# mpasha3/trips-py

Hardware: AMD Instinct MI355X
Metric: krylov_iters_per_sec (higher is better)
Workload: dtype f32; 1 GPU; blur4096_cgls; image=4096x4096 fp32, psf=Gaussian 9x9 sigma=(3,3), reflect, solver=CGLS (trips.solvers.CGLS semantics, tol=0), noise=1% Gaussian, parallelism=single

## Files before the change

include/trk.h:

```cpp
#ifndef TRK_H
#define TRK_H

#include <stdint.h>

#ifdef __cplusplus
extern "C" {
#endif

#define TRK_OK 0
#define TRK_EINVAL (-1)
#define TRK_EHIP (-2)
#define TRK_ENOMEM (-3)
#define TRK_EUNSUPPORTED (-4)
#define TRK_ENCCL (-5)

#define TRK_SQRT_NUM 1
#define TRK_SQRT_DEN 2

typedef struct trk_op trk_op;
typedef void* trk_stream;
typedef struct trk_comm trk_comm;

int trk_version(void);
const char* trk_last_error(void);
// ... 63 lines not shown
                    double* dot_out, trk_stream stream);
int trk_tv_grad_dot_xsq(trk_op* L, const float* x, const float* w, const float* r_in, double lam, float* out, const float* dotv,
                        double* dot_out, double* xsq_out, trk_stream stream);

#define TRK_HINT_OUT_FEEDS_OPPOSITE 1
#define TRK_HINT_INPUT_FROM_OPPOSITE 2
#define TRK_HINT_SUMSQ_DEFERRED 4
int trk_op_flush(trk_op* op, trk_stream stream);
int trk_op_axpby_caps(const trk_op* op, int* native);
int trk_op_apply_axpby(trk_op* op, int transpose, const float* x, double ca, const double* a_num, const double* a_den,
                       int a_flags, double cb, const double* b_num, const double* b_den, int b_flags, const float* z,
                       float* out, double* sumsq, int hints, trk_stream stream);

int trk_scalars_put(double* dst_dev, const double* src_host, int count, trk_stream stream);
typedef struct trk_mailbox trk_mailbox;
int trk_mailbox_create(int n_doubles, int slots, trk_mailbox** out);
int trk_mailbox_destroy(trk_mailbox* mb);
int trk_mailbox_host(trk_mailbox* mb, double** host_out);
int trk_mailbox_doubles(trk_mailbox* mb);
int trk_mailbox_slots(trk_mailbox* mb);
int trk_mailbox_post(trk_mailbox* mb, int slot, const double* src_dev, int offset, int count, trk_stream stream);
int trk_mailbox_wait(trk_mailbox* mb, int slot);
int trk_mailbox_post_sum(trk_mailbox* mb, int slot, const double* src_dev, int offset, int count, const double* partials,
                         int n_partials, double* sum_dev, int sum_offset, trk_stream stream);

int trk_gk_step(trk_op* op, int k, const float* u_k, const float* v_prev, float* v_k, float* u_next, double* AB, int chained,
                int defer_alpha, int defer_beta, trk_stream stream);
int trk_arnoldi_step(trk_op* op, float* V, int64_t ld, int k, float* w, double* G, int ldg, double* W, double* S, trk_stream stream);
int trk_arnoldi_step_post(trk_op* op, float* V, int64_t ld, int k, float* w, double* G, int ldg, double* W, double* S,
                          trk_mailbox* mb, int slot, int offset, int count, trk_stream stream);
int trk_arnoldi_step_post_at(trk_op* op, float* V, int64_t ld, int k, float* w, double* G, int ldg, double* W, double* S,
                             trk_mailbox* mb, int slot, int offset, int count, int host_offset, trk_stream stream);
int trk_arnoldi_step_post_dot(trk_op* op, float* V, int64_t ld, int k, float* w, double* G, int ldg, double* W, double* S,
                              trk_mailbox* mb, int slot, int offset, int count, int host_offset, const float* dotv, int dot_index,
                              trk_stream stream);
typedef struct trk_hgmres trk_hgmres;
typedef struct trk_host_worker trk_host_worker;
int trk_hgmres_create(trk_op* op, float* V, int64_t ld, int capacity, float* w, double* G, int ldg, double* W, double* S,
                      trk_mailbox* mb, trk_host_worker* const* workers, int n_workers, double beta0, trk_stream stream, trk_hgmres** out);
int trk_hgmres_destroy(trk_hgmres* g);
int trk_hgmres_start(trk_hgmres* g);
int trk_hgmres_iter(trk_hgmres* g, int absorb, int enqueue_next, int post_job, float* x_done, const float* ref, double* err_partials,
                    int err_cap, int* done_ii, double* done_lam, double* done_resid, int* done_blocks);
int trk_hgmres_hessenberg(trk_hgmres* g, double** H, int* ldh, int* columns);
int trk_hgmres_fixed_lambda(trk_hgmres* g, double lam);
int trk_hgmres_dp(trk_hgmres* g, const float* bvec, double bproj0, double target, double extra, double** bproj_out);
int trk_hgmres_stats(trk_hgmres* g, double* seconds5);
int trk_gk_step_post(trk_op* op, int k, const float* u_k, const float* v_prev, float* v_k, float* u_next, double* AB, int chained,
                     int defer_alpha, int defer_beta, const float* proj, double* proj_partials, int proj_cap, int* n_proj,
                     trk_mailbox* mb, int slot, const double* src_dev, int offset, int count, const double* sum_partials,
                     int n_sum, double* sum_dev, int sum_offset, trk_stream stream);
int trk_gk_step_lsqr(trk_op* op, int k, const float* u_k, const float* v_prev, float* v_k, float* u_next, double* AB, int chained,
                     int defer_alpha, int defer_beta, float* w, const float* x_in, float* x_out, const float* ref,
                     double* err_partials, int capacity_blocks, int* n_blocks, double damp, const double* state_in,
                     double* state_out, trk_stream stream);
int trk_gk_step_proj(trk_op* op, int k, const float* u_k, const float* v_prev, float* v_k, float* u_next, double* AB, int chained,
                     int defer_alpha, int defer_beta, const float* proj, double* partials, int cap, int* n_partials,
                     trk_stream stream);

int trk_cgls_update_xr(int64_t n, int64_t m, const double* gamma_dev, const double* delta_dev, const float* x,
                       const float* p, float* x_new, float* r, const float* w, const float* x_true,
                       double* sums_dev, trk_stream stream);

int trk_cgls_update_xr_deferred(int64_t n, int64_t m, const double* gamma_dev, const double* delta_dev, const float* x,
                                const float* p, float* x_new, float* r, const float* w, const float* x_true,
                                double* norm_partials, int capacity_blocks, int* n_blocks, trk_stream stream);
int trk_cgls_update_xr_src(int64_t n, int64_t m, const double* gamma, int gamma_n, const double* delta, int delta_n,
                           const float* x, const float* p, float* x_new, float* r, const float* w, const float* x_true,
                           double* publish_delta, double* norm_partials, int capacity_blocks, int* n_blocks,
                           trk_stream stream);
int trk_cgls_p_update(int64_t n, const float* t, float* p, const double* gamma_new, int gamma_new_n, const double* gamma_old,
                      double* publish_gamma, trk_stream stream);
int trk_cgls_update_grouping(int64_t n);
int trk_cgls_r_update(int64_t m, const double* gamma_old, const double* delta, int delta_n, float* r, const float* w,
                      double* publish_delta, trk_stream stream);
int trk_cgls_xp_update(int64_t n, const double* gamma_old, const double* delta, const double* gamma_new, int gamma_new_n,
                       const float* x, float* p, const float* t, float* x_new, const float* x_true, double* publish_gamma,
                       double* norm_partials, int capacity_blocks, int* n_blocks, trk_stream stream);
int trk_cgls_p_update_to(int64_t n, const float* t, const float* p, float* p_out, const double* gamma_new, int gamma_new_n,
                         const double* gamma_old, double* publish_gamma, trk_stream stream);
int trk_cgls_xs_update(int64_t n, int count, int k_last, double* S, const double* gamma_new, int gamma_new_n, const float* x,
                       const float* p, const float* ring, int64_t ring_ld, int s_slots, int first, const float* t, float* x_new,
                       float* p_out, const float* x_true, double* NP, int capacity_blocks, int* n_blocks, trk_stream stream);

int trk_op_fused_caps(const trk_op* op, int* can_fuse);
int trk_op_apply_fused(trk_op* op, int transpose, const float* x1, const float* x2, double sign, const double* num,
                       int num_n, const double* den, int den_n, float* comb_out, float* y, double* ysq_partials,
                       int capacity, int* n_partials, trk_stream stream);
int trk_cgls_x_update(int64_t n, const double* gamma, int gamma_n, const double* delta, int delta_n, const float* x,
                      const float* p, float* x_new, const float* x_true, double* publish_delta, double* publish_gamma,
                      double* norm_partials, int capacity_blocks, int* n_blocks, trk_stream stream);
int trk_bidiag_tikhonov(const double* alpha_sq, int64_t alpha_stride, const double* beta_sq, int64_t beta_stride, int k,
                        double mu, const double* beta0_sq, double* y, int y_over_alpha, double* work, int work_doubles,
                        trk_stream stream);
int trk_host_bidiag_tikhonov(const double* alpha, const double* beta_sub, int k, double beta0, double mu, int y_over_alpha, double* y);

int trk_host_gcv_fminbound(const double* s, const double* rhs, int k, double m_eff, double x1, double x2, double xatol,
                           int maxfun, double* lam_out, double* fval_out, int* nfev_out);
int trk_host_gcv_bidiag(const double* alpha, const double* beta, int k, double beta0, double m_eff, double x1, double x2,
                        double xatol, int maxfun, double* lam_out, double* fval_out, int* nfev_out);
int trk_host_dp_newton(const double* sv, const double* bhat, int n, double target, double extra, double* alpha_out,
                       int* alpha_set, int* iters_out);

int trk_host_dp_bidiag(const double* alpha, const double* beta_sub, int k, const double* bproj, double target, double extra,
                       double* alpha_out, int* alpha_set, int* iters_out, double* testzero_out);

typedef struct trk_host_worker trk_host_worker;
int trk_host_worker_create(trk_host_worker** out);
int trk_host_worker_destroy(trk_host_worker* w);
int trk_host_worker_post_gcv_bidiag(trk_host_worker* w, const double* alpha, const double* beta, int k, double beta0,
                                    double m_eff, double x1, double x2, double xatol, int maxfun);
int trk_host_worker_post_dp_bidiag(trk_host_worker* w, const double* alpha, const double* beta_sub, int k, const double* bproj,
                                   double target, double extra);
int trk_host_worker_collect(trk_host_worker* w, double* lam_out, int* have_out);
int trk_host_gram_gcv(void* const* lapack, const double* GA, const double* GL, int ldg, const double* c_select, const double* c_solve,
                      int k, double m_eff, double* lam_out, double* y_out, int* ok_out);
int trk_hlsqr_select(trk_host_worker* w, int mode, const double* alphas, const double* betas, int k_post, double beta0,
                     double m_eff_or_target, const double* bproj, double extra, int k_done, const float* V, int64_t ld, int64_t n,
                     float* x_out, const float* ref, double* err_partials, int err_cap, int* n_blocks, double* lam_out, int* have_out,
                     trk_stream stream);
int trk_host_worker_set_lapack(trk_host_worker* w, void* dgebrd, void* dormbr);
int trk_host_worker_post_hess_gcv(trk_host_worker* w, const double* H, int64_t h_row_stride, int64_t h_col_stride, int k,
                                  double beta0, double m_eff, double x1, double x2, double xatol, int maxfun);
int trk_host_worker_post_hess_fixed(trk_host_worker* w, const double* H, int64_t h_row_stride, int64_t h_col_stride, int k,
                                    double beta0, double lam);
int trk_host_worker_post_hess_dp(trk_host_worker* w, const double* H, int64_t h_row_stride, int64_t h_col_stride, int k,
                                 double beta0, const double* bproj, double target, double extra);
int trk_host_worker_collect_vec(trk_host_worker* w, double* lam_out, int* have_out, double* y, int k, double* resid_out);

int trk_cgls_iterate(trk_op* A, int k_first, int n_iters, float* p, float* r, float* t, float* w, float* X, int64_t x_ld,
                     int keep_history, const float* x_prev, const float* x_true, double* S, double* NP,
                     int np_capacity_blocks, int* n_np_inout, double* PG, double* PD, int pcap, int grouping,
                     trk_stream stream);
int trk_cgls_x_batch(int64_t n);
int trk_cgls_iterate_xbatch(trk_op* A, int k_first, int n_iters, float* p, float* ring, int64_t ring_ld, int s, float* r, float* t,
                            float* w, float* X, int64_t x_ld, const float* x_prev, const float* x_true, double* S, double* NP,
                            int np_capacity_blocks, int* n_np_inout, double* PG, double* PD, int pcap, trk_stream stream);
int trk_cgls_iterate_fused(trk_op* A, int k_first, int n_iters, float* P, int64_t p_ld, float* R, int64_t r_ld, float* t,
                           float* w, float* X, int64_t x_ld, int keep_history, const float* x_prev, const float* x_true,
                           double* S, double* PG, double* PD, int pcap, double* NP, int np_capacity_blocks,
                           int* n_g_inout, int* n_np_inout, trk_stream stream);

int trk_finalize_batched(const double* partials, int nblocks, int nvals, int batches, double* out, int out_stride,
                         trk_stream stream);

int trk_gemv_t(const float* V, int64_t ld, int k, int64_t n, const float* r, const float* w2, double* h_dev,
               trk_stream stream);
int trk_gemv_nt(const float* V, int64_t ld, int k, int64_t n, const double* h_dev, const float* w_in, float* w_out,
                double* g_dev, trk_stream stream);
int trk_gemv_t_x(const float* V, int64_t ld, int k, int64_t n, const float* r, const float* xrow, double* h, double* h_x,
                 trk_stream stream);
int trk_gemv_t2(const float* V, int64_t ld, int k, int64_t n, const float* r, const float* r2, double* h2k_dev,
                trk_stream stream);
int trk_cgs_coeffs(double* G_dev, int ldg, const double* h_dev, const double* g_new_dev, int k, int passes, double* c_dev,
                   trk_stream stream);
int trk_cgs_coeffs_rho(double* G_dev, int ldg, const double* h_dev, const double* g_new_dev, int k, int passes, double* c_dev,
                       const double* rr_dev, double* rho2_dev, trk_stream stream);
int trk_gemv_n(const float* V, int64_t ld, int k, int64_t n, const double* y_dev, double a, const float* base,
               double s, float* out, double* sumsq_dev, trk_stream stream);
int trk_gemv_n_err(const float* V, int64_t ld, int k, int64_t n, const double* y, float* out, const float* ref,
                   double* err_partials, int capacity_blocks, int* n_blocks, trk_stream stream);
int trk_gks_rows_solve(double* GA_dev, double* GL_dev, int ldg, int k, const double* ga_new, const double* a_A, const double* s_A,
                       const double* tb, const double* a_L, const double* s_L, const double* c_sweep, const double* rho2,
                       double* c_rhs, double lam, double* Minv, int ldm, int k_from, double* y, trk_stream stream);
int trk_gemv_orth_iterate(const float* V, int64_t ld, int k, int64_t n, const float* w, const double* c_dev, const double* rho2_dev,
                          const double* y_next_dev, float* vn, float* x_next, const float* ref, double* err_partials,
                          int capacity_blocks, int* n_blocks, double* chk_sumsq_dev, trk_stream stream);
int trk_gemv_n_hosty(const float* V, int64_t ld, int k, int64_t n, const double* y_host, float* out, const float* ref,
                     double* err_partials, int capacity_blocks, int* n_blocks, trk_stream stream);
int trk_lsqr_damped_update(const float* vk, float* w, const float* x_in, float* x_out, int64_t n, const float* ref,
                           double* err_partials, int capacity_blocks, int* n_blocks, const double* alpha_sq,
                           const double* beta_next_sq, const double* beta0_sq, double damp, const double* state_in,
                           double* state_out, int first, trk_stream stream);
int trk_radon2d_apply_ref(trk_op* op, int transpose, int elem_bytes, int weights, const void* x, void* y, trk_stream stream);
int trk_radon2d_set_arithmetic(trk_op* op, int mode);
int trk_radon2d_set_ref_sums(trk_op* op, int chunk_fwd, int chunk_adj);
int trk_ref_axpby(int elem_bytes, int64_t n, double ca, const double* a_num, const double* a_den, int a_flags, const void* x,
                  double cb, const double* b_num, const double* b_den, int b_flags, const void* z, void* out, double* sumsq,
                  trk_stream stream);
int trk_gk_lsqr_chain(trk_op* op, int elem_bytes, int weights, const void* b, int n_iter, double lambda, void* x_hist, void* work,
                      double* AB, double* state8, trk_stream stream);

int trk_wgram_tv(const float* V, int64_t ld, int k, int N, const float* w, double* G, trk_stream stream);
int trk_wgram_tv_precision(int mode);
int trk_wgram_tv_last_probe(double* verdict_and_deviation_host);
int trk_wgram_tv_z(const float* V, int64_t ld, int k, int N, const float* w, double* G, const float* z, double* h, trk_stream stream);

int trk_wgram(const float* W, int64_t ld, int k, int64_t m, const float* w, const float* b1, double* G_dev,
              double* c1_dev, double* c2_dev, trk_stream stream);

int trk_gemv_tn(const float* V, int64_t ld, int k, int64_t n, const float* const* rhs, int n_rhs, double* out_dev,
                trk_stream stream);
int trk_gram_row_from_sweep(double* G_dev, int ldg, int k, const double* a_dev, const double* c_dev, const double* s_rr_dev,
                            const double* rho2_dev, double* rhs_dev, const double* t_dev, trk_stream stream);

int trk_gram_tikhonov(const double* GA_dev, int lda, const double* GL_dev, int ldl, const double* c_dev, int k, double lam,
                      double* Minv_dev, int ldm, int k_from, double* y_dev, trk_stream stream);
int trk_hess_tikhonov(double* H_dev, int ldh, double* G_dev, double* Minv_dev, int ldg, const double* coef, const double* coef2,
                      const double* nrm2_sq, double beta0, int k, double lam, int mode, double* y_dev, trk_stream stream);

int trk_cgls_tiled_caps(trk_op* A, int np_capacity_blocks, int pcap, int* can);
int trk_cgls_iterate_tiled(trk_op* A, int k_first, int n_iters, float* P, int64_t p_ld, float* R, int64_t r_ld, float* t,
                           float* X, int64_t x_ld, int keep_history, const float* x_prev, const float* x_true, double* S,
                           double* PG, double* PD, int pcap, double* NP, int np_capacity_blocks, int* n_g_inout,
                           int* n_np_inout, trk_stream stream);

int trk_cgls_iterate_tiled2(trk_op* A, int k_first, int n_iters, float* p, float* w, float* R, int64_t r_ld, float* t, float* X,
                            int64_t x_ld, int keep_history, const float* x_prev, const float* x_true, double* S, double* PG,
                            double* PD, int pcap, double* NP, int np_capacity_blocks, int* n_g_inout, int* n_np_inout,
                            trk_stream stream);

int trk_comm_unique_id(void* id128_out);
int trk_comm_init(const void* id128, int rank, int world, trk_comm** out);
int trk_comm_attach(void* nccl_comm, int rank, int world, trk_comm** out);
int trk_comm_info(const trk_comm* comm, int* rank, int* world);
int trk_comm_destroy(trk_comm* comm);
int trk_allreduce_f64(trk_comm* comm, double* dev, int count, trk_stream stream);
int trk_halo_exchange(trk_comm* comm, const float* send, int send_to, float* recv, int recv_from, int64_t count,
                      trk_stream stream);
int trk_halo_exchange2(trk_comm* comm, const float* send_prev, float* recv_prev, const float* send_next, float* recv_next,
// ... 31 lines not shown
```

trips_py_amd/_lib.py:

```python
import ctypes
import os
import shutil
import subprocess
import sys
from concurrent.futures import ThreadPoolExecutor

HERE = os.path.dirname(os.path.abspath(__file__))
CSRC = os.path.join(HERE, "csrc")
INCLUDE = os.path.join(os.path.dirname(HERE), "include")
LIB_PATH = os.path.join(CSRC, "libtrk.so")
SOURCES = ["core.hip", "vecops.hip", "blur2d.hip", "gemv.hip", "wgram.hip", "tvops.hip", "radon2d.hip", "radon_fwd.hip", "radon_adj.hip", "spmv.hip", "framelet2d.hip", "fanbeam2d.hip", "projected.hip", "host_regparam.hip", "host_worker.hip", "hybrid_host.hip", "cgls_update.hip", "cgls_loop.hip", "comm.hip", "cgls_tiled.hip", "cgls_sharded.hip", "ref64.hip", "dense_svd.hip"]
HIPCC_FLAGS = ["-O3", "--offload-arch=gfx950", "-std=c++17", "-fPIC", "-I" + INCLUDE, "-I" + CSRC]


class TrkError(RuntimeError):
    pass


def _hipcc():
    exe = shutil.which("hipcc") or "/opt/rocm/bin/hipcc"
    if not os.path.exists(exe):
        raise TrkError("hipcc not found: cannot build libtrk.so (ROCm toolchain required)")
    return exe

# ... 112 lines not shown
    "trk_op_apply": (c_int, [c_op, c_int, c_f32p, c_i64, c_f32p, c_i64, c_int, c_f64p, c_stream]),
    "trk_op_destroy": (c_int, [c_op]),
    "trk_timer_create": (c_int, [c_int, ctypes.POINTER(ctypes.c_void_p)]),
    "trk_timer_reset": (c_int, [ctypes.c_void_p]),
    "trk_timer_read": (c_int, [ctypes.c_void_p, ctypes.POINTER(ctypes.c_float), c_int, ctypes.POINTER(c_int)]),
    "trk_timer_destroy": (c_int, [ctypes.c_void_p]),
    "trk_op_set_timer": (c_int, [c_op, ctypes.c_void_p, c_int]),
    "trk_dot": (c_int, [c_f32p, c_f32p, c_i64, c_f64p, c_stream]),
    "trk_nrm2sq": (c_int, [c_f32p, c_i64, c_f64p, c_stream]),
    "trk_diff_nrm2sq": (c_int, [c_f32p, c_f32p, c_i64, c_f64p, c_stream]),
    "trk_axpby": (c_int, [c_i64, c_dbl, c_f64p, c_f64p, c_int, c_f32p, c_dbl, c_f64p, c_f64p, c_int, c_f32p, c_f32p, c_f64p, c_stream]),
    "trk_scale_dot": (c_int, [c_i64, c_dbl, c_f64p, c_f64p, c_int, c_f32p, c_f32p, c_f32p, c_f64p, c_stream]),
    "trk_mul": (c_int, [c_i64, c_f32p, c_f32p, c_f32p, c_stream]),
    "trk_mul_diff": (c_int, [c_i64, c_f32p, c_f32p, c_f32p, c_f32p, c_stream]),
    "trk_group_weights": (c_int, [c_f32p, c_i64, c_int, c_dbl, c_dbl, c_int, c_f32p, c_stream]),
    "trk_isotv_weights": (c_int, [c_f32p, c_int, c_int, c_f32p, c_i64, c_dbl, c_dbl, c_f32p, c_stream]),
    "trk_tv_weights": (c_int, [c_op, c_f32p, c_dbl, c_dbl, c_f32p, c_stream]),
    "trk_arnoldi_step": (c_int, [c_op, c_f32p, c_i64, c_int, c_f32p, c_f64p, c_int, c_f64p, c_f64p, c_stream]),
    "trk_host_gram_gcv": (c_int, [ctypes.POINTER(ctypes.c_void_p), ctypes.c_void_p, ctypes.c_void_p, c_int, ctypes.c_void_p, ctypes.c_void_p,
                                 c_int, c_dbl, ctypes.POINTER(c_dbl), ctypes.c_void_p, ctypes.POINTER(c_int)]),
    "trk_hlsqr_select": (c_int, [ctypes.c_void_p, c_int, ctypes.c_void_p, ctypes.c_void_p, c_int, c_dbl, c_dbl, ctypes.c_void_p, c_dbl, c_int,
                                c_f32p, c_i64, c_i64, c_f32p, c_f32p, c_f64p, c_int, ctypes.POINTER(c_int), ctypes.POINTER(c_dbl),
                                ctypes.POINTER(c_int), c_stream]),
    "trk_hgmres_create": (c_int, [c_op, c_f32p, c_i64, c_int, c_f32p, c_f64p, c_int, c_f64p, c_f64p, ctypes.c_void_p,
                                 ctypes.POINTER(ctypes.c_void_p), c_int, c_dbl, c_stream,
                                 ctypes.POINTER(ctypes.c_void_p)]),
    "trk_hgmres_destroy": (c_int, [ctypes.c_void_p]),
    "trk_hgmres_start": (c_int, [ctypes.c_void_p]),
    "trk_hgmres_dp": (c_int, [ctypes.c_void_p, c_f32p, c_dbl, c_dbl, c_dbl, ctypes.POINTER(ctypes.POINTER(c_dbl))]),
    "trk_hgmres_fixed_lambda": (c_int, [ctypes.c_void_p, c_dbl]),
    "trk_hgmres_stats": (c_int, [ctypes.c_void_p, ctypes.POINTER(c_dbl)]),
    "trk_hgmres_iter": (c_int, [ctypes.c_void_p, c_int, c_int, c_int, c_f32p, c_f32p, c_f64p, c_int, ctypes.POINTER(c_int),
                               ctypes.POINTER(c_dbl), ctypes.POINTER(c_dbl), ctypes.POINTER(c_int)]),
    "trk_hgmres_hessenberg": (c_int, [ctypes.c_void_p, ctypes.POINTER(ctypes.POINTER(c_dbl)), ctypes.POINTER(c_int), ctypes.POINTER(c_int)]),
    "trk_arnoldi_step_post_dot": (c_int, [c_op, c_f32p, c_i64, c_int, c_f32p, c_f64p, c_int, c_f64p, c_f64p, ctypes.c_void_p, c_int, c_int, c_int,
                                         c_int, c_f32p, c_int, c_stream]),
    "trk_arnoldi_step_post_at": (c_int, [c_op, c_f32p, c_i64, c_int, c_f32p, c_f64p, c_int, c_f64p, c_f64p, ctypes.c_void_p, c_int, c_int, c_int,
                                        c_int, c_stream]),
    "trk_mailbox_doubles": (c_int, [ctypes.c_void_p]),
    "trk_mailbox_slots": (c_int, [ctypes.c_void_p]),
    "trk_host_worker_post_hess_fixed": (c_int, [ctypes.c_void_p, ctypes.c_void_p, c_i64, c_i64, c_int, c_dbl, c_dbl]),
    "trk_arnoldi_step_post": (c_int, [c_op, c_f32p, c_i64, c_int, c_f32p, c_f64p, c_int, c_f64p, c_f64p, ctypes.c_void_p, c_int, c_int, c_int,
                                     c_stream]),
    "trk_tv_grad": (c_int, [c_op, c_f32p, c_f32p, c_f32p, c_dbl, c_f32p, c_stream]),
    "trk_tv_halo": (c_int, [c_op, c_f32p, c_f32p]),
    "trk_tv_grad_dot": (c_int, [c_op, c_f32p, c_f32p, c_f32p, c_dbl, c_f32p, c_f32p, c_f64p, c_stream]),
    "trk_tv_grad_dot_xsq": (c_int, [c_op, c_f32p, c_f32p, c_f32p, c_dbl, c_f32p, c_f32p, c_f64p, c_f64p, c_stream]),
    "trk_mm_weights": (c_int, [c_i64, c_f32p, c_f32p, c_dbl, c_dbl, c_f32p, c_stream]),
    "trk_cgls_update_xr": (c_int, [c_i64, c_i64, c_f64p, c_f64p, c_f32p, c_f32p, c_f32p, c_f32p, c_f32p, c_f32p, c_f64p, c_stream]),
    "trk_op_fused_caps": (c_int, [c_op, ctypes.POINTER(c_int)]),
    "trk_op_axpby_caps": (c_int, [c_op, ctypes.POINTER(c_int)]),
    "trk_op_flush": (c_int, [c_op, c_stream]),
    "trk_op_apply_axpby": (c_int, [c_op, c_int, c_f32p, c_dbl, c_f64p, c_f64p, c_int, c_dbl, c_f64p, c_f64p, c_int, c_f32p,
                                   c_f32p, c_f64p, c_int, c_stream]),
    "trk_op_apply_fused": (c_int, [c_op, c_int, c_f32p, c_f32p, c_dbl, c_f64p, c_int, c_f64p, c_int, c_f32p, c_f32p, c_f64p, c_int, ctypes.POINTER(c_int), c_stream]),
    "trk_cgls_x_update": (c_int, [c_i64, c_f64p, c_int, c_f64p, c_int, c_f32p, c_f32p, c_f32p, c_f32p, c_f64p, c_f64p, c_f64p, c_int, ctypes.POINTER(c_int), c_stream]),
    "trk_finalize_batched": (c_int, [c_f64p, c_int, c_int, c_int, c_f64p, c_int, c_stream]),
    "trk_cgls_update_xr_deferred": (c_int, [c_i64, c_i64, c_f64p, c_f64p, c_f32p, c_f32p, c_f32p, c_f32p, c_f32p, c_f32p, c_f64p, c_int, ctypes.POINTER(c_int), c_stream]),
    "trk_bidiag_tikhonov": (c_int, [c_f64p, c_i64, c_f64p, c_i64, c_int, c_dbl, c_f64p, c_f64p, c_int, c_f64p, c_int,
                                   c_stream]),
    "trk_host_dp_newton": (c_int, [c_f64p, c_f64p, c_int, c_dbl, c_dbl, ctypes.POINTER(c_dbl), ctypes.POINTER(c_int),
                                  ctypes.POINTER(c_int)]),
    "trk_host_gcv_fminbound": (c_int, [c_f64p, c_f64p, c_int, c_dbl, c_dbl, c_dbl, c_dbl, c_int, ctypes.POINTER(c_dbl), ctypes.POINTER(c_dbl), ctypes.POINTER(c_int)]),
    "trk_host_dp_bidiag": (c_int, [c_f64p, c_f64p, c_int, c_f64p, c_dbl, c_dbl, ctypes.POINTER(c_dbl), ctypes.POINTER(c_int),
                                   ctypes.POINTER(c_int), ctypes.POINTER(c_dbl)]),
    "trk_host_gcv_bidiag": (c_int, [c_f64p, c_f64p, c_int, c_dbl, c_dbl, c_dbl, c_dbl, c_dbl, c_int, ctypes.POINTER(c_dbl),
                                    ctypes.POINTER(c_dbl), ctypes.POINTER(c_int)]),
    "trk_cgls_iterate": (c_int, [c_op, c_int, c_int, c_f32p, c_f32p, c_f32p, c_f32p, c_f32p, c_i64, c_int, c_f32p, c_f32p,
                                 c_f64p, c_f64p, c_int, ctypes.POINTER(c_int), c_f64p, c_f64p, c_int, c_int, c_stream]),
    "trk_cgls_update_xr_src": (c_int, [c_i64, c_i64, c_f64p, c_int, c_f64p, c_int, c_f32p, c_f32p, c_f32p, c_f32p, c_f32p,
                                       c_f32p, c_f64p, c_f64p, c_int, ctypes.POINTER(c_int), c_stream]),
    "trk_cgls_update_grouping": (c_int, [c_i64]),
    "trk_cgls_r_update": (c_int, [c_i64, c_f64p, c_f64p, c_int, c_f32p, c_f32p, c_f64p, c_stream]),
    "trk_cgls_xp_update": (c_int, [c_i64, c_f64p, c_f64p, c_f64p, c_int, c_f32p, c_f32p, c_f32p, c_f32p, c_f32p, c_f64p, c_f64p,
                                   c_int, ctypes.POINTER(c_int), c_stream]),
    "trk_cgls_p_update": (c_int, [c_i64, c_f32p, c_f32p, c_f64p, c_int, c_f64p, c_f64p, c_stream]),
    "trk_cgls_p_update_to": (c_int, [c_i64, c_f32p, c_f32p, c_f32p, c_f64p, c_int, c_f64p, c_f64p, c_stream]),
    "trk_cgls_xs_update": (c_int, [c_i64, c_int, c_int, c_f64p, c_f64p, c_int, c_f32p, c_f32p, c_f32p, c_i64, c_int, c_int, c_f32p,
                                   c_f32p, c_f32p, c_f32p, c_f64p, c_int, ctypes.POINTER(c_int), c_stream]),
    "trk_cgls_x_batch": (c_int, [c_i64]),
    "trk_cgls_iterate_xbatch": (c_int, [c_op, c_int, c_int, c_f32p, c_f32p, c_i64, c_int, c_f32p, c_f32p, c_f32p, c_f32p, c_i64,
                                        c_f32p, c_f32p, c_f64p, c_f64p, c_int, ctypes.POINTER(c_int), c_f64p, c_f64p, c_int,
                                        c_stream]),
    "trk_cgls_iterate_fused": (c_int, [c_op, c_int, c_int, c_f32p, c_i64, c_f32p, c_i64, c_f32p, c_f32p, c_f32p, c_i64, c_int,
                                       c_f32p, c_f32p, c_f64p, c_f64p, c_f64p, c_int, c_f64p, c_int, ctypes.POINTER(c_int),
                                       ctypes.POINTER(c_int), c_stream]),
    "trk_cgls_tiled_caps": (c_int, [c_op, c_int, c_int, ctypes.POINTER(c_int)]),
    "trk_cgls_iterate_tiled": (c_int, [c_op, c_int, c_int, c_f32p, c_i64, c_f32p, c_i64, c_f32p, c_f32p, c_i64, c_int,
                                       c_f32p, c_f32p, c_f64p, c_f64p, c_f64p, c_int, c_f64p, c_int, ctypes.POINTER(c_int),
                                       ctypes.POINTER(c_int), c_stream]),
    "trk_cgls_iterate_tiled2": (c_int, [c_op, c_int, c_int, c_f32p, c_f32p, c_f32p, c_i64, c_f32p, c_f32p, c_i64, c_int,
                                        c_f32p, c_f32p, c_f64p, c_f64p, c_f64p, c_int, c_f64p, c_int, ctypes.POINTER(c_int),
                                        ctypes.POINTER(c_int), c_stream]),
    "trk_gemv_t": (c_int, [c_f32p, c_i64, c_int, c_i64, c_f32p, c_f32p, c_f64p, c_stream]),
    "trk_gemv_t_x": (c_int, [c_f32p, c_i64, c_int, c_i64, c_f32p, c_f32p, c_f64p, c_f64p, c_stream]),
    "trk_gemv_t2": (c_int, [c_f32p, c_i64, c_int, c_i64, c_f32p, c_f32p, c_f64p, c_stream]),
    "trk_gemv_tn": (c_int, [c_f32p, c_i64, c_int, c_i64, ctypes.POINTER(ctypes.c_void_p), c_int, c_f64p, c_stream]),
    "trk_gram_row_from_sweep": (c_int, [c_f64p, c_int, c_int, c_f64p, c_f64p, c_f64p, c_f64p, c_f64p, c_f64p, c_stream]),
    "trk_gram_tikhonov": (c_int, [c_f64p, c_int, c_f64p, c_int, c_f64p, c_int, c_dbl, c_f64p, c_int, c_int, c_f64p, c_stream]),
    "trk_hess_tikhonov": (c_int, [c_f64p, c_int, c_f64p, c_f64p, c_int, c_f64p, c_f64p, c_f64p, c_dbl, c_int, c_dbl, c_int, c_f64p,
                                  c_stream]),
    "trk_cgs_coeffs": (c_int, [c_f64p, c_int, c_f64p, c_f64p, c_int, c_int, c_f64p, c_stream]),
    "trk_gks_rows_solve": (c_int, [c_f64p, c_f64p, c_int, c_int, c_f64p, c_f64p, c_f64p, c_f64p, c_f64p, c_f64p, c_f64p, c_f64p, c_f64p, c_dbl,
                                   c_f64p, c_int, c_int, c_f64p, c_stream]),
    "trk_cgs_coeffs_rho": (c_int, [c_f64p, c_int, c_f64p, c_f64p, c_int, c_int, c_f64p, c_f64p, c_f64p, c_stream]),
    "trk_gemv_orth_iterate": (c_int, [c_f32p, c_i64, c_int, c_i64, c_f32p, c_f64p, c_f64p, c_f64p, c_f32p, c_f32p, c_f32p, c_f64p, c_int,
                                      ctypes.POINTER(c_int), c_f64p, c_stream]),
    "trk_gemv_nt": (c_int, [c_f32p, c_i64, c_int, c_i64, c_f64p, c_f32p, c_f32p, c_f64p, c_stream]),
    "trk_gemv_n_err": (c_int, [c_f32p, c_i64, c_int, c_i64, c_f64p, c_f32p, c_f32p, c_f64p, c_int, ctypes.POINTER(c_int), c_stream]),
    "trk_host_worker_create": (c_int, [ctypes.POINTER(ctypes.c_void_p)]),
    "trk_host_worker_destroy": (c_int, [ctypes.c_void_p]),
    "trk_host_worker_post_gcv_bidiag": (c_int, [ctypes.c_void_p, ctypes.c_void_p, ctypes.c_void_p, c_int, c_dbl, c_dbl, c_dbl, c_dbl,
                                                c_dbl, c_int]),
    "trk_host_worker_post_dp_bidiag": (c_int, [ctypes.c_void_p, ctypes.c_void_p, ctypes.c_void_p, c_int, ctypes.c_void_p, c_dbl, c_dbl]),
    "trk_host_worker_collect": (c_int, [ctypes.c_void_p, ctypes.POINTER(c_dbl), ctypes.POINTER(c_int)]),
    "trk_host_worker_set_lapack": (c_int, [ctypes.c_void_p, ctypes.c_void_p, ctypes.c_void_p]),
    "trk_host_worker_post_hess_gcv": (c_int, [ctypes.c_void_p, ctypes.c_void_p, c_i64, c_i64, c_int, c_dbl, c_dbl, c_dbl, c_dbl, c_dbl, c_int]),
    "trk_host_worker_post_hess_dp": (c_int, [ctypes.c_void_p, ctypes.c_void_p, c_i64, c_i64, c_int, c_dbl, ctypes.c_void_p, c_dbl, c_dbl]),
    "trk_host_worker_collect_vec": (c_int, [ctypes.c_void_p, ctypes.POINTER(c_dbl), ctypes.POINTER(c_int), ctypes.c_void_p, c_int,
                                            ctypes.POINTER(c_dbl)]),
    "trk_scalars_put": (c_int, [c_f64p, ctypes.c_void_p, c_int, c_stream]),
    "trk_mailbox_create": (c_int, [c_int, c_int, ctypes.POINTER(ctypes.c_void_p)]),
    "trk_mailbox_destroy": (c_int, [ctypes.c_void_p]),
    "trk_mailbox_host": (c_int, [ctypes.c_void_p, ctypes.POINTER(ctypes.c_void_p)]),
    "trk_mailbox_post": (c_int, [ctypes.c_void_p, c_int, c_f64p, c_int, c_int, c_stream]),
    "trk_mailbox_wait": (c_int, [ctypes.c_void_p, c_int]),
    "trk_mailbox_post_sum": (c_int, [ctypes.c_void_p, c_int, c_f64p, c_int, c_int, c_f64p, c_int, c_f64p, c_int, c_stream]),
    "trk_gk_step_post": (c_int, [c_op, c_int, c_f32p, c_f32p, c_f32p, c_f32p, c_f64p, c_int, c_int, c_int, c_f32p, c_f64p, c_int,
                                 ctypes.POINTER(c_int), ctypes.c_void_p, c_int, c_f64p, c_int, c_int, c_f64p, c_int, c_f64p, c_int,
                                 c_stream]),
    "trk_gk_step_lsqr": (c_int, [c_op, c_int, c_f32p, c_f32p, c_f32p, c_f32p, c_f64p, c_int, c_int, c_int, c_f32p, c_f32p, c_f32p, c_f32p,
                                 c_f64p, c_int, ctypes.POINTER(c_int), c_dbl, c_f64p, c_f64p, c_stream]),
    "trk_gk_step_proj": (c_int, [c_op, c_int, c_f32p, c_f32p, c_f32p, c_f32p, c_f64p, c_int, c_int, c_int, c_f32p, c_f64p, c_int,
                                 ctypes.POINTER(c_int), c_stream]),
    "trk_host_bidiag_tikhonov": (c_int, [ctypes.c_void_p, ctypes.c_void_p, c_int, c_dbl, c_dbl, c_int, ctypes.c_void_p]),
    "trk_gemv_n_hosty": (c_int, [c_f32p, c_i64, c_int, c_i64, ctypes.c_void_p, c_f32p, c_f32p, c_f64p, c_int, ctypes.POINTER(c_int),
                                 c_stream]),
    "trk_gk_step": (c_int, [c_op, c_int, c_f32p, c_f32p, c_f32p, c_f32p, c_f64p, c_int, c_int, c_int, c_stream]),
    "trk_wgram_tv_precision": (c_int, [c_int]),
    "trk_wgram_tv_last_probe": (c_int, [ctypes.POINTER(c_dbl)]),
    "trk_radon2d_apply_ref": (c_int, [c_op, c_int, c_int, c_int, ctypes.c_void_p, ctypes.c_void_p, c_stream]),
    "trk_radon2d_set_arithmetic": (c_int, [c_op, c_int]),
    "trk_radon2d_set_ref_sums": (c_int, [c_op, c_int, c_int]),
    "trk_ref_axpby": (c_int, [c_int, c_i64, c_dbl, c_f64p, c_f64p, c_int, ctypes.c_void_p, c_dbl, c_f64p, c_f64p, c_int, ctypes.c_void_p,
                              ctypes.c_void_p, c_f64p, c_stream]),
    "trk_gk_lsqr_chain": (c_int, [c_op, c_int, c_int, ctypes.c_void_p, c_int, c_dbl, ctypes.c_void_p, ctypes.c_void_p, c_f64p, c_f64p,
                                  c_stream]),
    "trk_lsqr_damped_update": (c_int, [c_f32p, c_f32p, c_f32p, c_f32p, c_i64, c_f32p, c_f64p, c_int, ctypes.POINTER(c_int),
                                       c_f64p, c_f64p, c_f64p, c_dbl, c_f64p, c_f64p, c_int, c_stream]),
    "trk_gemv_n": (c_int, [c_f32p, c_i64, c_int, c_i64, c_f64p, c_dbl, c_f32p, c_dbl, c_f32p, c_f64p, c_stream]),
    "trk_comm_unique_id": (c_int, [ctypes.c_void_p]),
    "trk_comm_init": (c_int, [ctypes.c_void_p, c_int, c_int, ctypes.POINTER(ctypes.c_void_p)]),
    "trk_comm_attach": (c_int, [ctypes.c_void_p, c_int, c_int, ctypes.POINTER(ctypes.c_void_p)]),
    "trk_comm_info": (c_int, [ctypes.c_void_p, ctypes.POINTER(c_int), ctypes.POINTER(c_int)]),
    "trk_comm_destroy": (c_int, [ctypes.c_void_p]),
    "trk_allreduce_f64": (c_int, [ctypes.c_void_p, c_f64p, c_int, c_stream]),
    "trk_halo_exchange": (c_int, [ctypes.c_void_p, c_f32p, c_int, c_f32p, c_int, c_i64, c_stream]),
    "trk_halo_exchange2": (c_int, [ctypes.c_void_p, c_f32p, c_f32p, c_f32p, c_f32p, c_i64, c_stream]),
    "trk_dot_pair": (c_int, [c_f32p, c_f32p, c_i64, c_f64p, c_stream]),
    "trk_cgls_sharded_update": (c_int, [c_i64, c_i64, c_f64p, c_f64p, c_int, c_f32p, c_f32p, c_f32p, c_f32p, c_f32p, c_f32p,
                                        c_f32p, c_f32p, c_f64p, c_f64p, c_f64p, c_int, ctypes.POINTER(c_int), c_stream]),
    "trk_cgls_sharded_scalars": (c_int, [c_f32p, c_f32p, c_i64, c_f64p, c_int, c_f64p, c_stream]),
    "trk_cgls_iterate_sharded": (c_int, [c_op, ctypes.c_void_p, c_int, c_int, c_f32p, c_f32p, c_f32p, c_f32p, c_f32p, c_f32p, c_i64,
                                         c_int, c_f32p, c_f32p, c_f64p, c_f64p, c_f64p, c_int, ctypes.POINTER(c_int), c_f64p, c_int,
                                         ctypes.POINTER(c_int), c_stream]),
    "trk_wgram_tv_z": (c_int, [c_f32p, c_i64, c_int, c_int, c_f32p, c_f64p, c_f32p, c_f64p, c_stream]),
# ... 56 lines not shown
```

trips_py_amd/csrc/blur2d.hip:

```cpp
#include "trk_internal.h"
#include <hip/hip_ext.h>

#include <cmath>
#include <cstdlib>
#include <type_traits>
#include <vector>

using namespace trk;

namespace {

constexpr int NT = 256;
constexpr int TW = 128;
constexpr int TH = 32;

typedef float f4 __attribute__((ext_vector_type(4)));

__host__ __device__ constexpr int rup4(int v) { return (v + 3) & ~3; }

__device__ __forceinline__ int reflect(int i, int n) {
  if ((unsigned)i < (unsigned)n) return i;
  const int p = 2 * n;
  i %= p;
  if (i < 0) i += p;
// ... 166 lines not shown
        }
      } else {
#pragma unroll
        for (int rr = 0; rr < 4; ++rr) {
          if (a - rr >= 0 && a - rr < KH) {
#pragma unroll
            for (int b = 0; b < KW; ++b) {
              const float w = wts[(a - rr) * KW + b];
#pragma unroll
              for (int c = 0; c < 4; ++c) acc[rr][c] = fmaf(w, v[OFF + c + b], acc[rr][c]);
            }
          }
        }
      }
    }

    if (vec_ok) {
#pragma unroll
      for (int rr = 0; rr < 4; ++rr) {
        const int gi = i0 + 4 * ty + rr;
        if (gi < i_end) {
          *reinterpret_cast<f4*>(y + (int64_t)gi * ny + gj) = (f4){acc[rr][0], acc[rr][1], acc[rr][2], acc[rr][3]};
          if (SUMSQ)
            ss += (double)acc[rr][0] * acc[rr][0] + (double)acc[rr][1] * acc[rr][1] +
                  (double)acc[rr][2] * acc[rr][2] + (double)acc[rr][3] * acc[rr][3];
        }
      }
    } else {
#pragma unroll
      for (int rr = 0; rr < 4; ++rr) {
        const int gi = i0 + 4 * ty + rr;
        if (gi < i_end) {
#pragma unroll
          for (int c = 0; c < 4; ++c)
            if (gj + c < ny) {
              y[(int64_t)gi * ny + gj + c] = acc[rr][c];
              if (SUMSQ) ss += (double)acc[rr][c] * acc[rr][c];
            }
        }
      }
    }

    if (has_next) {
      __syncthreads();
#pragma unroll
      for (int q = 0; q < NPF; ++q) {
        const int idx = threadIdx.x + q * NT;
        if (idx < TH * SW4) {
          const int r = idx / SW4, c4 = idx - r * SW4;
          S4[((rel_base + RING + r) % RING) * SW4 + c4] = pf[q];
        }
      }
      rb += TH;
      if (rb >= RING) rb -= RING;
    }
  }
  if (SUMSQ) {
    ss = block_sum<NT>(ss, red);
    if (threadIdx.x == 0) partials[(size_t)blockIdx.y * gridDim.x + blockIdx.x] = ss;
  }
}

typedef unsigned int u4 __attribute__((ext_vector_type(4)));
typedef float f2 __attribute__((ext_vector_type(2)));

__host__ __device__ constexpr int gcd_c(int a, int b) { return b == 0 ? a : gcd_c(b, a % b); }
__host__ __device__ constexpr int lcm_c(int a, int b) { return a / gcd_c(a, b) * b; }
__host__ __device__ constexpr int pmod(int a, int m) { return ((a % m) + m) % m; }

constexpr int SPAN = 256;

struct SlideFuse {
  const float* x2;
  float* comb;
  double sign;
  ScalarSrc num, den;
};

struct SlideEpi {
  const float* z;
  Coef a, b;
};

template <int KH, int KW, int D, bool SUMSQ, bool FUSE, bool EPI = false, int BC = BC_REFLECT>
__global__ __launch_bounds__(64) void k_blur_slide(const float* __restrict__ x, int64_t ldx, float* __restrict__ y,
                                                   int64_t ldy, int nx, int ny, const float* __restrict__ wts,
                                                   double* __restrict__ partials, int spans_x, int nbands,
                                                   int rows_per_band, SlideFuse fz, int nt_store, SlideEpi ep = SlideEpi{}) {
  constexpr int T = KH - 1 - KH / 2;
  constexpr int Lh = KW - 1 - KW / 2;
  constexpr int OFFC = 4 - Lh;
  constexpr int U = lcm_c(KH, D);
  static_assert(Lh <= 4 && KW / 2 <= 4, "sliding kernel handles halos of at most one 4-column group");

  int band, span;
  {
    const int id = blockIdx.x, total = nbands * spans_x;
    const int xcd = id & 7, local = id >> 3;
    const int t = xcd * (total >> 3) + min(xcd, total & 7) + local;
    band = t / spans_x;
    span = t - band * spans_x;
  }
  x += (int64_t)blockIdx.y * ldx;
  y += (int64_t)blockIdx.y * ldy;
  const int i_begin = band * rows_per_band;
  const int i_end = (i_begin + rows_per_band < nx) ? i_begin + rows_per_band : nx;
  const int lane = threadIdx.x;
  const int c0 = span * SPAN + 4 * lane;
  const bool active = c0 < ny;
  const int cc = active ? c0 : ny - 4;
  const int cl = (BC == BC_WRAP && c0 == 0) ? ny - 4 : (cc >= 4) ? cc - 4 : 0;
  const int cr = (BC == BC_WRAP && c0 + 4 == ny) ? 0 : (cc + 8 <= ny) ? cc + 4 : ny - 4;
  const bool ledge = (c0 == 0), redge = (c0 + 4 == ny);
  const bool edge_span = (span == 0) || ((span + 1) * SPAN >= ny);

  const unsigned img_bytes = (unsigned)nx * (unsigned)ny * 4u;
  const auto rin = __builtin_amdgcn_make_buffer_rsrc((void*)x, 0, img_bytes, 0x00020000);
  const auto rout = __builtin_amdgcn_make_buffer_rsrc((void*)y, 0, img_bytes, 0x00020000);
  const auto rin2 = __builtin_amdgcn_make_buffer_rsrc((void*)(FUSE ? fz.x2 : x), 0, img_bytes, 0x00020000);
  const auto rcomb = __builtin_amdgcn_make_buffer_rsrc((void*)(FUSE ? fz.comb : y), 0, img_bytes, 0x00020000);
  float cb = 0.f;
  if (FUSE) cb = (fz.sign == 0.0) ? 0.f : (float)(fz.sign * scalar_from_wave(fz.num, threadIdx.x) / scalar_from_wave(fz.den, threadIdx.x));
  const int vl = cl * 4, vr = cr * 4;
  const int vc = cc * 4;
  const int vst = c0 * 4;

  const bool up = (band & 1) != 0;
  float wr[KW], wc[KH];
#pragma unroll
  for (int b = 0; b < KW; ++b) wr[b] = wts[b];
#pragma unroll
  for (int a = 0; a < KH; ++a) wc[a] = up ? wts[KW + KH - 1 - a] : wts[KW + a];

  const int band_rows = i_end - i_begin;
  const int total = ((band_rows + KH - 1 + U - 1) / U) * U;
  const int rowbytes = ny * 4;
  const int dir = up ? -1 : 1;
  const int first = up ? (i_end - 1 + KH / 2) : (i_begin - T);
  const int last = first + dir * (total - 1);
  const bool interior = (first >= 0) && (first < nx) && (last >= 0) && (last < nx);
  const int ofirst = up ? (i_end - 1) : i_begin;

  f4 pL[D], pC[D], pR[D];
  f4 qL[FUSE ? D : 1], qC[FUSE ? D : 1], qR[FUSE ? D : 1];
  auto issue = [&](int t, int slot) {
    int gi = first + dir * t;
    if (!interior) gi = bmap<BC>(gi, nx);
    if constexpr (BC == BC_CONSTANT) {
      if (gi < 0) {
        const f4 z = (f4){0.f, 0.f, 0.f, 0.f};
        pL[slot] = pC[slot] = pR[slot] = z;
        if (FUSE) qL[slot] = qC[slot] = qR[slot] = z;
        return;
      }
    }
    const int so = gi * rowbytes;
    pL[slot] = __builtin_bit_cast(f4, __builtin_amdgcn_raw_buffer_load_b128(rin, vl, so, 0));
    pC[slot] = __builtin_bit_cast(f4, __builtin_amdgcn_raw_buffer_load_b128(rin, vc, so, 0));
    pR[slot] = __builtin_bit_cast(f4, __builtin_amdgcn_raw_buffer_load_b128(rin, vr, so, 0));
    if (FUSE) {
      qL[slot] = __builtin_bit_cast(f4, __builtin_amdgcn_raw_buffer_load_b128(rin2, vl, so, 0));
      qC[slot] = __builtin_bit_cast(f4, __builtin_amdgcn_raw_buffer_load_b128(rin2, vc, so, 0));
      qR[slot] = __builtin_bit_cast(f4, __builtin_amdgcn_raw_buffer_load_b128(rin2, vr, so, 0));
    }
  };
#pragma unroll
  for (int d = 0; d < D; ++d) issue(d, d);
  float ea = 1.f, eb = 0.f;
  f4 zq[EPI ? D : 1];
  const auto rz = __builtin_amdgcn_make_buffer_rsrc((void*)((EPI && ep.z) ? ep.z : x), 0, img_bytes, 0x00020000);
  const bool has_z = EPI && ep.z != nullptr;
  auto issue_z = [&](int o, int slot) {
    const int oc = o < band_rows - 1 ? o : band_rows - 1;
    zq[slot] = __builtin_bit_cast(f4, __builtin_amdgcn_raw_buffer_load_b128(rz, vc, (ofirst + dir * oc) * rowbytes, 0));
  };
  if (EPI) {
    ea = (float)coef_eval(ep.a);
    eb = has_z ? (float)coef_eval(ep.b) : 0.f;
    if (has_z) {
#pragma unroll
      for (int d = 0; d < D; ++d) issue_z(d, d);
    }
  }

  f2 acc[KH][2];
  double ss = 0.0;
  float qacc = 0.f;

  auto block = [&](int t0, auto guard_tag) {
    constexpr bool GUARD = decltype(guard_tag)::value;
#pragma unroll
    for (int u = 0; u < U; ++u) {
      const int t = t0 + u;
      const int slot = u % D;
      f4 Lv = pL[slot], Cv = pC[slot], Rv = pR[slot];
      if (FUSE) {
        Lv = Lv + cb * qL[slot];
        Cv = Cv + cb * qC[slot];
        Rv = Rv + cb * qR[slot];
        const int graw = first + dir * t;
        if (graw >= i_begin && graw < i_end && active)
          __builtin_amdgcn_raw_buffer_store_b128(__builtin_bit_cast(u4, Cv), rcomb, vst + graw * rowbytes, 0, 0);
      }
      if (!GUARD || t + D < total) issue(t + D, slot);
      if constexpr (BC == BC_REFLECT) {
        if (edge_span) {
          const f4 rev = (f4){Cv[3], Cv[2], Cv[1], Cv[0]};
          if (ledge) Lv = rev;
          if (redge) Rv = rev;
        }
      } else if constexpr (BC != BC_WRAP) {
        if (edge_span) {
          f4 le, re;
          if constexpr (BC == BC_CONSTANT) {
            le = re = (f4){0.f, 0.f, 0.f, 0.f};
          } else if constexpr (BC == BC_NEAREST) {
            le = (f4){Cv[0], Cv[0], Cv[0], Cv[0]};
            re = (f4){Cv[3], Cv[3], Cv[3], Cv[3]};
          } else {
            le = (f4){Rv[0], Cv[3], Cv[2], Cv[1]};
            re = (f4){Cv[2], Cv[1], Cv[0], Lv[3]};
          }
          if (ledge) Lv = le;
          if (redge) Rv = re;
        }
      }
      const float v[12] = {Lv[0], Lv[1], Lv[2], Lv[3], Cv[0], Cv[1], Cv[2], Cv[3], Rv[0], Rv[1], Rv[2], Rv[3]};
      float h0 = 0.f, h1 = 0.f, h2 = 0.f, h3 = 0.f;
#pragma unroll
      for (int b = 0; b < KW; ++b) {
        h0 = fmaf(wr[b], v[OFFC + b], h0);
        h1 = fmaf(wr[b], v[OFFC + b + 1], h1);
        h2 = fmaf(wr[b], v[OFFC + b + 2], h2);
        h3 = fmaf(wr[b], v[OFFC + b + 3], h3);
      }
      const f2 hlo = {h0, h1}, hhi = {h2, h3};
#pragma unroll
      for (int a = 0; a < KH; ++a) {
        const int k = pmod(u - a, KH);
        if (a == 0) {
          acc[k][0] = wc[0] * hlo;
          acc[k][1] = wc[0] * hhi;
        } else {
          acc[k][0] = wc[a] * hlo + acc[k][0];
          acc[k][1] = wc[a] * hhi + acc[k][1];
        }
      }
      const int o = t - (KH - 1);
      if (!GUARD || (o >= 0 && o < band_rows)) {
        const int kd = pmod(u - (KH - 1), KH);
        f4 out = (f4){acc[kd][0][0], acc[kd][0][1], acc[kd][1][0], acc[kd][1][1]};
        if (EPI) {
          const int zs = pmod(u - (KH - 1), D);
          if (has_z) {
            const f4 zv = zq[zs];
#pragma unroll
            for (int e = 0; e < 4; ++e) out[e] = fmaf(ea, out[e], eb * zv[e]);
            issue_z(o + D, zs);
          } else {
#pragma unroll
            for (int e = 0; e < 4; ++e) out[e] = ea * out[e];
          }
        }
        if (active) {
          if (nt_store & 1)
            __builtin_amdgcn_raw_buffer_store_b128(__builtin_bit_cast(u4, out), rout, vst + (ofirst + dir * o) * rowbytes, 0, 2);
          else
            __builtin_amdgcn_raw_buffer_store_b128(__builtin_bit_cast(u4, out), rout, vst + (ofirst + dir * o) * rowbytes, 0, 0);
          if (SUMSQ) qacc = fmaf(out[0], out[0], fmaf(out[1], out[1], fmaf(out[2], out[2], fmaf(out[3], out[3], qacc))));
        }
      }
      if (SUMSQ && (u & 3) == 3) {
        ss += (double)qacc;
        qacc = 0.f;
      }
    }
  };
  block(0, std::true_type{});
  int t0 = U;
  for (; t0 + U < total; t0 += U) block(t0, std::false_type{});
  if (t0 < total) block(t0, std::true_type{});
  if (SUMSQ) ss += (double)qacc;
  if (SUMSQ) {
    ss = wave_sum(ss);
    if (lane == 0) partials[(size_t)blockIdx.y * gridDim.x + blockIdx.x] = ss;
  }
}

template <bool SUMSQ, int BC = BC_REFLECT>
__global__ __launch_bounds__(NT) void k_blur_generic(const float* __restrict__ x, int64_t ldx, float* __restrict__ y,
                                                     int64_t ldy, int nx, int ny, int kh, int kw,
                                                     const float* __restrict__ w, double* __restrict__ partials) {
  __shared__ double red[NT / 64];
  const int T = kh - 1 - kh / 2, L = kw - 1 - kw / 2;
  x += (int64_t)blockIdx.y * ldx;
  y += (int64_t)blockIdx.y * ldy;
  const int64_t npix = (int64_t)nx * ny;
  double ss = 0.0;
  for (int64_t idx = (int64_t)blockIdx.x * NT + threadIdx.x; idx < npix; idx += (int64_t)gridDim.x * NT) {
    const int i = (int)(idx / ny), j = (int)(idx - (int64_t)i * ny);
    float acc = 0.f;
    for (int a = 0; a < kh; ++a) {
      const int gi = bmap<BC>(i - T + a, nx);
      if constexpr (BC == BC_CONSTANT)
        if (gi < 0) continue;
      const float* row = x + (int64_t)gi * ny;
      for (int b = 0; b < kw; ++b) acc = fmaf(w[a * kw + b], bload<BC>(row, j - L + b, ny), acc);
    }
    y[idx] = acc;
    if (SUMSQ) ss += (double)acc * acc;
  }
  if (SUMSQ) {
    ss = block_sum<NT>(ss, red);
    if (threadIdx.x == 0) partials[(size_t)blockIdx.y * gridDim.x + blockIdx.x] = ss;
  }
}

inline void strip_grid(int nx, int ny, int batch, int* strips_x, int* rows_per_band, int* nband) {
  const int sx = ceil_div(ny, TW), steps = ceil_div(nx, TH);
  int want = (4 * cu_count()) / (sx * (batch > 0 ? batch : 1));
  if (want < 1) want = 1;
  if (want > steps) want = steps;
  const int steps_per_band = ceil_div(steps, want);
  *strips_x = sx;
  *rows_per_band = steps_per_band * TH;
  *nband = ceil_div(nx, *rows_per_band);
}

template <int K, int BC>
int launch_strip(const BlurImpl* im, int tr, const float* x, int64_t ldx, float* y, int64_t ldy, int batch,
                 double* part, int strips_x, int rows_per_band, int nband, hipStream_t s) {
  dim3 grid(strips_x * nband, batch), block(NT);
  const float* w = im->separable ? im->sep_dev[tr] : im->w_dev[tr];
#define BL(SEP, SS) \
  hipLaunchKernelGGL((k_blur_strip<K, K, SEP, SS, BC>), grid, block, 0, s, x, ldx, y, ldy, im->nx, im->ny, w, part, strips_x, rows_per_band)
  if (im->separable) { if (part) BL(true, true); else BL(true, false); }
  else               { if (part) BL(false, true); else BL(false, false); }
#undef BL
  TRK_LAUNCH_CHECK();
  return TRK_OK;
}

template <int K, int D, int BC>
int launch_slide(const BlurImpl* im, int tr, const float* x, int64_t ldx, float* y, int64_t ldy, int batch,
                 double* part, int spans_x, int nbands, int rows_per_band, hipStream_t s, hipEvent_t ev0, hipEvent_t ev1,
                 const SlideFuse* fuse = nullptr, const SlideEpi* epi = nullptr) {
  dim3 grid(spans_x * nbands, batch), block(64);
  const float* w = im->sep_dev[tr];
  const int nts = stream_nontemporal((int64_t)im->nx * im->ny);
  if (fuse) {
    hipExtLaunchKernelGGL((k_blur_slide<K, K, D, true, true, false, BC>), grid, block, 0, s, ev0, ev1, 0, x, ldx, y, ldy, im->nx, im->ny, w, part, spans_x, nbands, rows_per_band, *fuse, nts, SlideEpi{});
    TRK_LAUNCH_CHECK();
    return TRK_OK;
  }
  const SlideFuse nofuse{nullptr, nullptr, 0.0, {nullptr, 0}, {nullptr, 0}};
  if (epi) {
    if (part)
      hipExtLaunchKernelGGL((k_blur_slide<K, K, D, true, false, true, BC>), grid, block, 0, s, ev0, ev1, 0, x, ldx, y, ldy, im->nx, im->ny, w, part, spans_x, nbands, rows_per_band, nofuse, nts, *epi);
    else
      hipExtLaunchKernelGGL((k_blur_slide<K, K, D, false, false, true, BC>), grid, block, 0, s, ev0, ev1, 0, x, ldx, y, ldy, im->nx, im->ny, w, part, spans_x, nbands, rows_per_band, nofuse, nts, *epi);
    TRK_LAUNCH_CHECK();
    return TRK_OK;
  }
  if (part)
    hipExtLaunchKernelGGL((k_blur_slide<K, K, D, true, false, false, BC>), grid, block, 0, s, ev0, ev1, 0, x, ldx, y, ldy, im->nx, im->ny, w, part, spans_x, nbands, rows_per_band, nofuse, nts, SlideEpi{});
  else
    hipExtLaunchKernelGGL((k_blur_slide<K, K, D, false, false, false, BC>), grid, block, 0, s, ev0, ev1, 0, x, ldx, y, ldy, im->nx, im->ny, w, part, spans_x, nbands, rows_per_band, nofuse, nts, SlideEpi{});
  TRK_LAUNCH_CHECK();
  return TRK_OK;
}

inline void slide_grid(int nx, int ny, int batch, int kh, int U, int* spans_x, int* nbands, int* rows_per_band) {
  const int sx = ceil_div(ny, SPAN);
  const double slots = 4.0 * cu_count();
  const int nb = batch > 0 ? batch : 1;
  int rows = U;
  while (rows - (kh - 1) < kh + 1) rows += U;
  int rpb = rows - (kh - 1);
  double best = 1e300;
  for (;; rows += U) {
    const int r = rows - (kh - 1);
    const double x = (double)sx * ceil_div(nx, r) * nb / slots;
    const double g = x <= 1.0 ? 1.0 : 0.6 + 0.45 * x + 0.5 * (ceil(x) - 1.0);
    const bool last = x <= 1.0 || r >= nx;
    if ((x * slots <= 3840.0 || last) && rows * g < best) {
      best = rows * g;
      rpb = r;
    }
    if (last) break;
  }
  *spans_x = sx;
  *nbands = ceil_div(nx, rpb);
  *rows_per_band = rpb;
}

inline bool slide_shape_ok(const BlurImpl* im) {
  return im->separable && im->kh == im->kw && (im->kh & 1) && im->kh >= 3 && im->kh <= 9 && (im->ny & 3) == 0 &&
         im->ny >= 8 && (int64_t)im->nx * im->ny < ((int64_t)1 << 29);
}

int blur_apply_fused(trk_op* op, int tr, const float* x1, const float* x2, double sign, ScalarSrc num, ScalarSrc den,
                     float* comb, float* y, double* partials, int cap, int* n_partials, hipStream_t s) {
  auto* im = static_cast<BlurImpl*>(op->impl);
  if (!slide_shape_ok(im) || !aligned16(x1) || !aligned16(y) || (x2 && (!aligned16(x2) || !aligned16(comb))))
    return fail(TRK_EUNSUPPORTED, "blur2d fused apply: needs a separable odd PSF <= 9x9, ny %% 4 == 0, 16-byte aligned buffers");
  if (x2 && (comb == x1 || comb == x2))
    return fail(TRK_EINVAL, "blur2d fused apply: comb must not alias an input (halo rows are shared)");
  int spans_x, nbands, rpb;
  const int Usel = (im->kh == 9) ? 9 : (im->kh == 7) ? 7 : (im->kh == 5) ? 5 : 6;
  slide_grid(im->nx, im->ny, 1, im->kh, Usel, &spans_x, &nbands, &rpb);
  const int nblk = spans_x * nbands;
  if (nblk > cap) return fail(TRK_EINVAL, "blur2d fused apply: partial buffer holds %d doubles, %d needed", cap, nblk);
  *n_partials = nblk;
  const SlideFuse fz{x2, comb, sign, num, den};
  const SlideFuse* fzp = x2 ? &fz : nullptr;
  hipEvent_t ev0 = nullptr, ev1 = nullptr;
  if (trk_timer* t = op->timer)
    if ((op->timer_which == 2 || op->timer_which == tr) && t->used < t->cap) {
      ev0 = t->ev[2 * t->used];
      ev1 = t->ev[2 * t->used + 1];
      ++t->used;
    }
  return bc_dispatch(im->bc, [&](auto bc) {
    constexpr int BC = decltype(bc)::value;
    switch (im->kh) {
      case 3: return launch_slide<3, 6, BC>(im, tr, x1, 0, y, 0, 1, partials, spans_x, nbands, rpb, s, ev0, ev1, fzp);
      case 5: return launch_slide<5, 5, BC>(im, tr, x1, 0, y, 0, 1, partials, spans_x, nbands, rpb, s, ev0, ev1, fzp);
      case 7: return launch_slide<7, 7, BC>(im, tr, x1, 0, y, 0, 1, partials, spans_x, nbands, rpb, s, ev0, ev1, fzp);
      default:
        return launch_slide<9, 9, BC>(im, tr, x1, 0, y, 0, 1, partials, spans_x, nbands, rpb, s, ev0, ev1, fzp);
    }
  });
}

int blur_apply(trk_op* op, int tr, const float* x, int64_t ldx, float* y, int64_t ldy, int batch, double* sumsq,
               hipStream_t s) {
  auto* im = static_cast<BlurImpl*>(op->impl);
  double* part = nullptr;
  int nblk;
  const bool slide_ok = slide_shape_ok(im) && aligned16(x) && aligned16(y) &&
                        (batch == 1 || ((ldx & 3) == 0 && (ldy & 3) == 0));
  if (slide_ok) {
    int spans_x, nbands, rpb;
    const int Usel = (im->kh == 9) ? 9 : (im->kh == 7) ? 7 : (im->kh == 5) ? 5 : 6;
    slide_grid(im->nx, im->ny, batch, im->kh, Usel, &spans_x, &nbands, &rpb);
    nblk = spans_x * nbands;
    if (sumsq)
      if (int rc = scratch_doubles(s, (size_t)nblk * batch, &part)) return rc;
    hipEvent_t ev0 = nullptr, ev1 = nullptr;
    if (trk_timer* t = op->timer)
// ... 14 lines not shown
    if (rc) return rc;
    if (sumsq) return finalize_sums(part, nblk * batch, 1, 1, sumsq, s);
    return TRK_OK;
  }
  if (im->tiled) {
    int strips_x, rows_per_band, nband;
    strip_grid(im->nx, im->ny, batch, &strips_x, &rows_per_band, &nband);
    nblk = strips_x * nband;
    if (sumsq)
      if (int rc = scratch_doubles(s, (size_t)nblk * batch, &part)) return rc;
    TimerScope tm(op->timer, op->timer_which, tr, s);
    const int rc = bc_dispatch(im->bc, [&](auto bc) {
      constexpr int BC = decltype(bc)::value;
      switch (im->kh) {
        case 3: return launch_strip<3, BC>(im, tr, x, ldx, y, ldy, batch, part, strips_x, rows_per_band, nband, s);
        case 5: return launch_strip<5, BC>(im, tr, x, ldx, y, ldy, batch, part, strips_x, rows_per_band, nband, s);
        case 7: return launch_strip<7, BC>(im, tr, x, ldx, y, ldy, batch, part, strips_x, rows_per_band, nband, s);
        case 9: return launch_strip<9, BC>(im, tr, x, ldx, y, ldy, batch, part, strips_x, rows_per_band, nband, s);
        case 11: return launch_strip<11, BC>(im, tr, x, ldx, y, ldy, batch, part, strips_x, rows_per_band, nband, s);
        case 13: return launch_strip<13, BC>(im, tr, x, ldx, y, ldy, batch, part, strips_x, rows_per_band, nband, s);
        case 15: return launch_strip<15, BC>(im, tr, x, ldx, y, ldy, batch, part, strips_x, rows_per_band, nband, s);
        default: return fail(TRK_EUNSUPPORTED, "blur2d: no strip kernel for %dx%d", im->kh, im->kw);
      }
    });
    tm.stop();
    if (rc) return rc;
  } else {
    const int64_t npix = (int64_t)im->nx * im->ny;
    int64_t want = (npix + NT - 1) / NT;
    if (want > 4096) want = 4096;
    nblk = (int)(want < 1 ? 1 : want);
    if (sumsq)
      if (int rc = scratch_doubles(s, (size_t)nblk * batch, &part)) return rc;
    dim3 grid(nblk, batch);
    TimerScope tm(op->timer, op->timer_which, tr, s);
    bc_dispatch(im->bc, [&](auto bc) {
      constexpr int BC = decltype(bc)::value;
      if (part)
        hipLaunchKernelGGL((k_blur_generic<true, BC>), grid, dim3(NT), 0, s, x, ldx, y, ldy, im->nx, im->ny, im->kh, im->kw, im->w_dev[tr], part);
      else
        hipLaunchKernelGGL((k_blur_generic<false, BC>), grid, dim3(NT), 0, s, x, ldx, y, ldy, im->nx, im->ny, im->kh, im->kw, im->w_dev[tr], part);
      return 0;
    });
    tm.stop();
    TRK_LAUNCH_CHECK();
  }
  if (sumsq) return finalize_sums(part, nblk * batch, 1, 1, sumsq, s);
  return TRK_OK;
}

int blur_apply_axpby_plain(trk_op* op, int tr, const float* x, Coef a, Coef b, const float* z, float* out, double* sumsq,
                           hipStream_t s) {
  auto* im = static_cast<BlurImpl*>(op->impl);
  if (!slide_shape_ok(im) || !aligned16(x) || !aligned16(out) || (z && !aligned16(z))) return TRK_EUNSUPPORTED;
  int spans_x, nbands, rpb;
  const int Usel = (im->kh == 9) ? 9 : (im->kh == 7) ? 7 : (im->kh == 5) ? 5 : 6;
  slide_grid(im->nx, im->ny, 1, im->kh, Usel, &spans_x, &nbands, &rpb);
  const int nblk = spans_x * nbands;
  double* part = nullptr;
  if (sumsq)
    if (int rc = scratch_doubles(s, (size_t)nblk, &part)) return rc;
  hipEvent_t ev0 = nullptr, ev1 = nullptr;
  if (trk_timer* t = op->timer)
    if ((op->timer_which == 2 || op->timer_which == tr) && t->used < t->cap) {
      ev0 = t->ev[2 * t->used];
      ev1 = t->ev[2 * t->used + 1];
      ++t->used;
    }
  const SlideEpi ep{z, a, b};
  const int rc = bc_dispatch(im->bc, [&](auto bc) {
    constexpr int BC = decltype(bc)::value;
    switch (im->kh) {
      case 3: return launch_slide<3, 6, BC>(im, tr, x, 0, out, 0, 1, part, spans_x, nbands, rpb, s, ev0, ev1, nullptr, &ep);
      case 5: return launch_slide<5, 5, BC>(im, tr, x, 0, out, 0, 1, part, spans_x, nbands, rpb, s, ev0, ev1, nullptr, &ep);
      case 7: return launch_slide<7, 7, BC>(im, tr, x, 0, out, 0, 1, part, spans_x, nbands, rpb, s, ev0, ev1, nullptr, &ep);
      default: return launch_slide<9, 9, BC>(im, tr, x, 0, out, 0, 1, part, spans_x, nbands, rpb, s, ev0, ev1, nullptr, &ep);
    }
  });
  if (rc) return rc;
  if (sumsq) return finalize_sums(part, nblk, 1, 1, sumsq, s);
  return TRK_OK;
}

void blur_destroy(trk_op* op) {
  auto* im = static_cast<BlurImpl*>(op->impl);
  for (int t = 0; t < 2; ++t) {
    if (im->w_dev[t]) (void)hipFree(im->w_dev[t]);
    if (im->sep_dev[t]) (void)hipFree(im->sep_dev[t]);
  }
  delete im;
}

}

namespace trk {
bool blur_separable_params(trk_op* op, int* nx, int* ny, int* kh, int* kw, const float** sep_fwd, const float** sep_adj,
                           int* boundary) {
  if (!op || op->kind != 1) return false;
  auto* im = static_cast<BlurImpl*>(op->impl);
  if (!im->separable || !im->sep_dev[0] || !im->sep_dev[1]) return false;
  if (boundary) *boundary = im->bc;
  *nx = im->nx;
  *ny = im->ny;
  *kh = im->kh;
  *kw = im->kw;
  *sep_fwd = im->sep_dev[0];
  *sep_adj = im->sep_dev[1];
  return true;
}
}

extern "C" int trk_blur2d_create(const double* psf, int kh, int kw, int nx, int ny, trk_op** out) {
  return trk_blur2d_create_bc(psf, kh, kw, nx, ny, TRK_BOUNDARY_REFLECT, out);
}

extern "C" int trk_blur2d_create_bc(const double* psf, int kh, int kw, int nx, int ny, int boundary, trk_op** out) {
  TRK_REQUIRE(psf && out, "trk_blur2d_create: NULL argument");
  TRK_REQUIRE(kh >= 1 && kw >= 1 && nx >= 1 && ny >= 1, "trk_blur2d_create: sizes must be >= 1");
  TRK_REQUIRE((int64_t)kh * kw <= (1 << 24), "trk_blur2d_create: PSF too large");
  TRK_REQUIRE(boundary >= TRK_BOUNDARY_REFLECT && boundary <= TRK_BOUNDARY_WRAP, "trk_blur2d_create_bc: unknown boundary mode %d", boundary);
  static_assert(TRK_BOUNDARY_REFLECT == BC_REFLECT && TRK_BOUNDARY_CONSTANT == BC_CONSTANT && TRK_BOUNDARY_NEAREST == BC_NEAREST &&
                    TRK_BOUNDARY_MIRROR == BC_MIRROR && TRK_BOUNDARY_WRAP == BC_WRAP,
                "blur2d boundary modes follow trk.h");
  auto* im = new BlurImpl{nx, ny, kh, kw, boundary, false, false, {nullptr, nullptr}, {nullptr, nullptr}};

  std::vector<float> wf((size_t)kh * kw), wt((size_t)kh * kw);
  for (int a = 0; a < kh; ++a)
    for (int b = 0; b < kw; ++b) {
      wf[(size_t)a * kw + b] = (float)psf[(size_t)(kh - 1 - a) * kw + (kw - 1 - b)];
      wt[(size_t)a * kw + b] = (float)psf[(size_t)a * kw + b];
    }

  int pa = 0, pb = 0;
  double pmax = 0.0;
  for (int a = 0; a < kh; ++a)
    for (int b = 0; b < kw; ++b)
      if (std::fabs(psf[(size_t)a * kw + b]) > pmax) {
        pmax = std::fabs(psf[(size_t)a * kw + b]);
        pa = a;
        pb = b;
      }
  std::vector<double> col(kh), row(kw);
  bool sep = pmax > 0.0;
  if (sep) {
    const double piv = psf[(size_t)pa * kw + pb];
    for (int a = 0; a < kh; ++a) col[a] = psf[(size_t)a * kw + pb];
    for (int b = 0; b < kw; ++b) row[b] = psf[(size_t)pa * kw + b] / piv;
    for (int a = 0; a < kh && sep; ++a)
      for (int b = 0; b < kw; ++b)
        if (std::fabs(psf[(size_t)a * kw + b] - col[a] * row[b]) > 1e-12 * pmax) {
          sep = false;
          break;
        }
  }
  im->separable = sep;
  im->tiled = (kh == kw) && (kh & 1) && kh >= 3 && kh <= 15;

  auto upload = [](const std::vector<float>& h, float** d) -> int {
    TRK_HIP(hipMalloc(d, h.size() * sizeof(float)));
    TRK_HIP(hipMemcpy(*d, h.data(), h.size() * sizeof(float), hipMemcpyHostToDevice));
    return TRK_OK;
  };
  int rc = upload(wf, &im->w_dev[0]);
  if (!rc) rc = upload(wt, &im->w_dev[1]);
  if (!rc && sep) {
    std::vector<float> sf(kw + kh), st(kw + kh);
    for (int b = 0; b < kw; ++b) {
      sf[b] = (float)row[kw - 1 - b];
      st[b] = (float)row[b];
    }
    for (int a = 0; a < kh; ++a) {
      sf[kw + a] = (float)col[kh - 1 - a];
      st[kw + a] = (float)col[a];
    }
    rc = upload(sf, &im->sep_dev[0]);
    if (!rc) rc = upload(st, &im->sep_dev[1]);
  }
  if (rc) {
    trk_op tmp{1, 0, 0, im, nullptr, nullptr, nullptr, 0};
    blur_destroy(&tmp);
    return rc;
  }
  const int64_t n = (int64_t)nx * ny;
  auto* op = new trk_op{1, n, n, im, blur_apply, blur_destroy, nullptr, 0};
  if (slide_shape_ok(im)) op->apply_fused = blur_apply_fused;
  if (slide_shape_ok(im)) op->apply_axpby_plain = blur_apply_axpby_plain;
  *out = op;
  return TRK_OK;
}
```

trips_py_amd/csrc/cgls_loop.hip:

```cpp
#include "trk_internal.h"

using namespace trk;

extern "C" {

int trk_cgls_update_grouping(int64_t n) {
  return n >= ((int64_t)8 << 20) ? 1 : 0;
}

int trk_cgls_iterate(trk_op* A, int k_first, int n_iters, float* p, float* r, float* t, float* w, float* X, int64_t x_ld,
                     int keep_history, const float* x_prev, const float* x_true, double* S, double* NP,
                     int np_capacity_blocks, int* n_np_inout, double* PG, double* PD, int pcap, int grouping,
                     trk_stream stream) {
  TRK_REQUIRE(A && p && r && t && w && X && x_prev && S && NP && n_np_inout, "trk_cgls_iterate: NULL argument");
  TRK_REQUIRE(k_first >= 1 && n_iters >= 0, "trk_cgls_iterate: need k_first >= 1, n_iters >= 0");
  const int64_t m = A->rows, n = A->cols;
  int n_np = *n_np_inout;
  const bool raw = PG && PD && pcap > 0 && A->apply_fused;
  const bool xp_form = (grouping < 0 ? trk_cgls_update_grouping(n) : grouping) == 1;
  for (int k = k_first; k < k_first + n_iters; ++k) {
    double* row = S + 5 * (int64_t)k;
    double *delta = row, *gamma = row + 1;
    const double* gamma_old = (k == 1) ? S : row - 4;
    float* x_new = X + (int64_t)(keep_history ? (k - 1) : ((k - 1) & 1)) * x_ld;
// ... 8 lines not shown
      if (rc) return rc;
      rc = trk_cgls_xp_update(n, gamma_old, delta, PG, n_g, x_prev, p, t, x_new, x_true, gamma,
                              NP + 3 * (int64_t)n_np * (k - 1), np_capacity_blocks, &n_np, stream);
      if (rc) return rc;
      x_prev = x_new;
      continue;
    }
    if (raw) {
      int n_d = 0, n_g = 0;
      rc = trk_op_apply_fused(A, 0, p, nullptr, 0.0, nullptr, 0, nullptr, 0, nullptr, w, PD, pcap, &n_d, stream);
      if (rc) return rc;
      rc = trk_cgls_update_xr_src(n, m, gamma_old, 1, PD, n_d, x_prev, p, x_new, r, w, x_true, delta,
                                  NP + 3 * (int64_t)n_np * (k - 1), np_capacity_blocks, &n_np, stream);
      if (rc) return rc;
      rc = trk_op_apply_fused(A, 1, r, nullptr, 0.0, nullptr, 0, nullptr, 0, nullptr, t, PG, pcap, &n_g, stream);
      if (rc) return rc;
      rc = trk_cgls_p_update(n, t, p, PG, n_g, gamma_old, gamma, stream);
      if (rc) return rc;
      x_prev = x_new;
      continue;
    }
    rc = trk_op_apply(A, 0, p, 0, w, 0, 1, delta, stream);
    if (rc) return rc;
    rc = trk_cgls_update_xr_deferred(n, m, gamma_old, delta, x_prev, p, x_new, r, w, x_true,
                                     NP + 3 * (int64_t)n_np * (k - 1), np_capacity_blocks, &n_np, stream);
    if (rc) return rc;
    rc = trk_op_apply(A, 1, r, 0, t, 0, 1, gamma, stream);
    if (rc) return rc;
    rc = trk_axpby(n, 1.0, nullptr, nullptr, 0, t, 1.0, gamma, gamma_old, 0, p, p, nullptr, stream);
    if (rc) return rc;
    x_prev = x_new;
  }
  *n_np_inout = n_np;
  return TRK_OK;
}

int trk_cgls_x_batch(int64_t n) {
  return n >= ((int64_t)8 << 20) ? 8 : 1;
}

int trk_cgls_iterate_xbatch(trk_op* A, int k_first, int n_iters, float* p, float* ring, int64_t ring_ld, int s, float* r, float* t,
                            float* w, float* X, int64_t x_ld, const float* x_prev, const float* x_true, double* S, double* NP,
                            int np_capacity_blocks, int* n_np_inout, double* PG, double* PD, int pcap, trk_stream stream) {
  TRK_REQUIRE(A && p && r && t && w && X && x_prev && S && NP && n_np_inout && PG && PD && pcap > 0,
              "trk_cgls_iterate_xbatch: NULL argument");
  TRK_REQUIRE(A->apply_fused, "trk_cgls_iterate_xbatch: the operator has no fused apply (trk_op_fused_caps)");
  TRK_REQUIRE(k_first >= 1 && n_iters >= 0, "trk_cgls_iterate_xbatch: need k_first >= 1, n_iters >= 0");
  TRK_REQUIRE(s >= 1 && (s == 1 || (ring && ring_ld >= A->cols)), "trk_cgls_iterate_xbatch: s > 1 needs a ring of s - 1 directions");
  const int64_t m = A->rows, n = A->cols;
  int n_np = *n_np_inout;
  auto slot = [&](int j) { return j == 0 ? p : ring + (int64_t)(j - 1) * ring_ld; };
  int cur = 0, pending = 0;
  const int k_end = k_first + n_iters;
  for (int k = k_first; k < k_end; ++k) {
    double* row = S + 5 * (int64_t)k;
    const double* gamma_old = (k == 1) ? S : row - 4;
    float* p_k = slot(cur);
    int n_d = 0, n_g = 0;
    int rc = trk_op_apply_fused(A, 0, p_k, nullptr, 0.0, nullptr, 0, nullptr, 0, nullptr, w, PD, pcap, &n_d, stream);
    if (rc) return rc;
    rc = trk_cgls_r_update(m, gamma_old, PD, n_d, r, w, row, stream);
    if (rc) return rc;
    rc = trk_op_apply_fused(A, 1, r, nullptr, 0.0, nullptr, 0, nullptr, 0, nullptr, t, PG, pcap, &n_g, stream);
    if (rc) return rc;
    const bool last = k + 1 == k_end;
    if (++pending < s && !last) {
      cur = (cur + 1) % s;
      rc = trk_cgls_p_update_to(n, t, p_k, slot(cur), PG, n_g, gamma_old, row + 1, stream);
      if (rc) return rc;
      continue;
    }
    float* x_new = X + (int64_t)((k - 1) & 1) * x_ld;
    rc = trk_cgls_xs_update(n, pending, k, S, PG, n_g, x_prev, p, ring, ring_ld, s, (cur - pending + 1 + s) % s, t, x_new,
                            last ? p : p_k, x_true, NP, np_capacity_blocks, &n_np, stream);
    if (rc) return rc;
    x_prev = x_new;
    pending = 0;
    if (last) cur = 0;
  }
  *n_np_inout = n_np;
  return TRK_OK;
}

int trk_cgls_iterate_fused(trk_op* A, int k_first, int n_iters, float* P, int64_t p_ld, float* R, int64_t r_ld, float* t,
                           float* w, float* X, int64_t x_ld, int keep_history, const float* x_prev, const float* x_true,
                           double* S, double* PG, double* PD, int pcap, double* NP, int np_capacity_blocks,
                           int* n_g_inout, int* n_np_inout, trk_stream stream) {
  TRK_REQUIRE(A && P && R && t && w && X && x_prev && S && PG && PD && NP && n_g_inout && n_np_inout,
              "trk_cgls_iterate_fused: NULL argument");
  TRK_REQUIRE(k_first >= 1 && n_iters >= 0, "trk_cgls_iterate_fused: need k_first >= 1, n_iters >= 0");
  const int64_t n = A->cols;
  int n_g = *n_g_inout, n_np = *n_np_inout, n_d = 0;
  for (int k = k_first; k < k_first + n_iters; ++k) {
    const int64_t b = 5 * (int64_t)k;
    float *p_old = P + (int64_t)((k - 1) & 1) * p_ld, *p_new = P + (int64_t)(k & 1) * p_ld;
    float *r_old = R + (int64_t)((k - 1) & 1) * r_ld, *r_new = R + (int64_t)(k & 1) * r_ld;
    const double* gprev = (k <= 2) ? S : S + 5 * (int64_t)(k - 2) + 1;
    int rc = trk_op_apply_fused(A, 0, t, p_old, k == 1 ? 0.0 : 1.0, PG, n_g, gprev, 1, p_new, w, PD, pcap, &n_d, stream);
    if (rc) return rc;
    float* x_new = X + (int64_t)(keep_history ? (k - 1) : ((k - 1) & 1)) * x_ld;
    double* gpub = (k == 1) ? S : S + b - 4;
    rc = trk_cgls_x_update(n, PG, n_g, PD, n_d, x_prev, p_new, x_new, x_true, S + b, gpub,
                           NP + 3 * (int64_t)n_np * (k - 1), np_capacity_blocks, &n_np, stream);
    if (rc) return rc;
    rc = trk_op_apply_fused(A, 1, r_old, w, -1.0, gpub, 1, S + b, 1, r_new, t, PG, pcap, &n_g, stream);
    if (rc) return rc;
    x_prev = x_new;
  }
  *n_g_inout = n_g;
  *n_np_inout = n_np;
  return TRK_OK;
}

}
```

trips_py_amd/csrc/cgls_update.hip:

```cpp
#include "vec_internal.h"

using namespace trk;

namespace {

__device__ __forceinline__ float x_step(float x, float p, float step, float& d) {
  d = step * p;
  return x + d;
}
__device__ __forceinline__ float4 x_step4(float4 xv, float4 pv, float step, float4& d) {
  d = make_float4(step * pv.x, step * pv.y, step * pv.z, step * pv.w);
  return make_float4(xv.x + d.x, xv.y + d.y, xv.z + d.z, xv.w + d.w);
}
template <bool HAS_XT>
__device__ __forceinline__ void x_norms(float xn, float d, float xt, double& s0, double& s1, double& s2) {
  s0 += (double)xn * xn;
  s1 += (double)d * d;
  if (HAS_XT) {
    const double e = (double)xn - xt;
    s2 += e * e;
  }
}
template <bool HAS_XT>
__device__ __forceinline__ void x_norms4(float4 xn, float4 d, float4 tt, double& s0, double& s1, double& s2) {
// ... 111 lines not shown
template <bool VEC>
__global__ __launch_bounds__(NT) void k_cgls_r_update(int64_t m, const double* gold, ScalarSrc delta, float* r,
                                                      const float* __restrict__ w, double* pub_delta) {
  __shared__ double bc;
  if (threadIdx.x < 64) {
    const double d = scalar_from_wave(delta, threadIdx.x);
    if (threadIdx.x == 0) {
      bc = *gold / d;
      if (blockIdx.x == 0 && pub_delta) *pub_delta = d;
    }
  }
  __syncthreads();
  const float step = (float)bc;
  const int64_t tid = (int64_t)blockIdx.x * NT + threadIdx.x, nth = (int64_t)gridDim.x * NT;
  int64_t tail0 = 0;
  if (VEC) {
    const int64_t m4 = m >> 2;
    tail0 = m4 << 2;
    for (int64_t i = tid; i < m4; i += nth) {
      float4 rv = ld4(r, i);
      const float4 wv = ld4(w, i);
      rv.x = fmaf(-step, wv.x, rv.x);
      rv.y = fmaf(-step, wv.y, rv.y);
      rv.z = fmaf(-step, wv.z, rv.z);
      rv.w = fmaf(-step, wv.w, rv.w);
      st4(r, i, rv);
    }
  }
  for (int64_t i = tail0 + tid; i < m; i += nth) r[i] = fmaf(-step, w[i], r[i]);
}

template <bool HAS_XT>
__global__ __launch_bounds__(NT) void k_cgls_xp_update(int64_t n, const double* gold, const double* delta, ScalarSrc gnew,
                                                       const float* __restrict__ x, float* p, const float* __restrict__ t,
                                                       float* __restrict__ x_new, const float* __restrict__ x_true,
                                                       double* pub_gamma, double* __restrict__ partials, int nt) {
  __shared__ double lds[NT / 64];
  __shared__ double bc[2];
  if (threadIdx.x < 64) {
    const double g = scalar_from_wave(gnew, threadIdx.x);
    if (threadIdx.x == 0) {
      bc[0] = *gold / *delta;
      bc[1] = g / *gold;
      if (blockIdx.x == 0 && pub_gamma) *pub_gamma = g;
    }
  }
  __syncthreads();
  const float step = (float)bc[0], b = (float)bc[1];
  double s0 = 0.0, s1 = 0.0, s2 = 0.0;
  const int64_t tid = (int64_t)blockIdx.x * NT + threadIdx.x, nth = (int64_t)gridDim.x * NT;
  const int64_t n4 = n >> 2;
  for (int64_t i = tid; i < n4; i += nth) {
    const float4 xv = (nt & 16) ? ld4_nt(x, i) : ld4(x, i), pv = ld4(p, i), tv = (nt & 32) ? ld4_nt(t, i) : ld4(t, i);
    float4 d;
    const float4 xn = x_step4(xv, pv, step, d);
    if (nt & 2) st4_nt(x_new, i, xn); else st4(x_new, i, xn);
    st4(p, i, p_step4(tv, pv, b));
    x_norms4<HAS_XT>(xn, d, HAS_XT ? ld4(x_true, i) : make_float4(0.f, 0.f, 0.f, 0.f), s0, s1, s2);
  }
  for (int64_t i = (n4 << 2) + tid; i < n; i += nth) {
    const float pv = p[i];
    float d;
    const float xn = x_step(x[i], pv, step, d);
    x_new[i] = xn;
    p[i] = fmaf(1.f, t[i], b * pv);
    x_norms<HAS_XT>(xn, d, HAS_XT ? x_true[i] : 0.f, s0, s1, s2);
  }
  s0 = block_sum<NT>(s0, lds);
  s1 = block_sum<NT>(s1, lds);
  if (HAS_XT) s2 = block_sum<NT>(s2, lds);
  if (threadIdx.x == 0) {
    partials[blockIdx.x * 3 + 0] = s0;
    partials[blockIdx.x * 3 + 1] = s1;
    partials[blockIdx.x * 3 + 2] = HAS_XT ? s2 : 0.0;
  }
}

constexpr int kXsOldDirs = 256 | 32, kXsLastDirAndOut = 512 | 1024;
constexpr int XS_MAX = 8;
struct XsDirs {
  const float* p[XS_MAX];
};

template <bool HAS_XT, int C>
__global__ __launch_bounds__(NT) void k_cgls_xs_update(int64_t n, const double* S, int k, ScalarSrc gnew, const float* x, XsDirs dirs,
                                                       const float* __restrict__ t, float* x_new, float* p_out,
                                                       const float* __restrict__ x_true, double* pub_gamma,
                                                       double* __restrict__ partials, int64_t slice, int nt) {
  __shared__ double lds[NT / 64];
  __shared__ double bc[C + 1];
  if (threadIdx.x < 64) {
    const double g = scalar_from_wave(gnew, threadIdx.x);
    if (threadIdx.x == 0) {
#pragma unroll
      for (int c = 0; c < C; ++c) {
        const int j = k - C + 1 + c;
        const double* gold = (j == 1) ? S : S + 5 * (int64_t)(j - 1) + 1;
        bc[c] = *gold / S[5 * (int64_t)j];
      }
      bc[C] = g / *((k == 1) ? S : S + 5 * (int64_t)(k - 1) + 1);
      if (blockIdx.x == 0 && pub_gamma) *pub_gamma = g;
    }
  }
  __syncthreads();
  float step[C];
#pragma unroll
  for (int c = 0; c < C; ++c) step[c] = (float)bc[c];
  const float b = (float)bc[C];
  double s0[C], s1[C], s2[C];
#pragma unroll
  for (int c = 0; c < C; ++c) s0[c] = s1[c] = s2[c] = 0.0;
  const int64_t tid = (int64_t)blockIdx.x * NT + threadIdx.x, nth = (int64_t)gridDim.x * NT;
  const int64_t n4 = n >> 2;
  for (int64_t i = tid; i < n4; i += nth) {
    float4 xv = (nt & 16) ? ld4_nt(x, i) : ld4(x, i);
    float4 pv[C];
#pragma unroll
    for (int c = 0; c < C; ++c) pv[c] = (nt & (c < C - 1 ? 256 : 512)) ? ld4_nt(dirs.p[c], i) : ld4(dirs.p[c], i);
    const float4 tv = (nt & 32) ? ld4_nt(t, i) : ld4(t, i);
    const float4 tt = HAS_XT ? ld4(x_true, i) : make_float4(0.f, 0.f, 0.f, 0.f);
#pragma unroll
    for (int c = 0; c < C; ++c) {
      float4 d;
      xv = x_step4(xv, pv[c], step[c], d);
      x_norms4<HAS_XT>(xv, d, tt, s0[c], s1[c], s2[c]);
    }
    if (nt & 2) st4_nt(x_new, i, xv); else st4(x_new, i, xv);
    if (nt & 1024) st4_nt(p_out, i, p_step4(tv, pv[C - 1], b)); else st4(p_out, i, p_step4(tv, pv[C - 1], b));
  }
  for (int64_t i = (n4 << 2) + tid; i < n; i += nth) {
    float xv = x[i];
    float pv[C];
#pragma unroll
    for (int c = 0; c < C; ++c) pv[c] = dirs.p[c][i];
    const float tv = t[i], tt = HAS_XT ? x_true[i] : 0.f;
#pragma unroll
    for (int c = 0; c < C; ++c) {
      float d;
      xv = x_step(xv, pv[c], step[c], d);
      x_norms<HAS_XT>(xv, d, tt, s0[c], s1[c], s2[c]);
    }
    x_new[i] = xv;
    p_out[i] = fmaf(1.f, tv, b * pv[C - 1]);
  }
#pragma unroll
  for (int c = 0; c < C; ++c) {
    const double a0 = block_sum<NT>(s0[c], lds), a1 = block_sum<NT>(s1[c], lds);
    const double a2 = HAS_XT ? block_sum<NT>(s2[c], lds) : 0.0;
    if (threadIdx.x == 0) {
      double* out = partials + c * slice + blockIdx.x * 3;
      out[0] = a0;
      out[1] = a1;
      out[2] = a2;
    }
  }
}

template <bool HAS_XT>
__global__ __launch_bounds__(NT) void k_cgls_x_update(int64_t n, ScalarSrc gamma, ScalarSrc delta, const float* __restrict__ x,
                                                      const float* __restrict__ p, float* __restrict__ x_new,
                                                      const float* __restrict__ x_true, double* pub_delta,
                                                      double* pub_gamma, double* __restrict__ partials) {
  __shared__ double lds[NT / 64];
  __shared__ double bc[2];
  if (threadIdx.x < 64) {
    const double g = scalar_from_wave(gamma, threadIdx.x), d = scalar_from_wave(delta, threadIdx.x);
    if (threadIdx.x == 0) {
      bc[0] = g;
      bc[1] = d;
      if (blockIdx.x == 0) {
        if (pub_gamma) *pub_gamma = g;
        if (pub_delta) *pub_delta = d;
      }
    }
  }
  __syncthreads();
  const float step = (float)(bc[0] / bc[1]);
  double s0 = 0.0, s1 = 0.0, s2 = 0.0;
  const int64_t tid = (int64_t)blockIdx.x * NT + threadIdx.x, nth = (int64_t)gridDim.x * NT;
  const int64_t n4 = n >> 2;
  for (int64_t i = tid; i < n4; i += nth) {
    const float4 xv = ld4(x, i), pv = ld4(p, i);
    const float4 d = make_float4(step * pv.x, step * pv.y, step * pv.z, step * pv.w);
    const float4 xn = make_float4(xv.x + d.x, xv.y + d.y, xv.z + d.z, xv.w + d.w);
    st4(x_new, i, xn);
    s0 += (double)xn.x * xn.x + (double)xn.y * xn.y + (double)xn.z * xn.z + (double)xn.w * xn.w;
    s1 += (double)d.x * d.x + (double)d.y * d.y + (double)d.z * d.z + (double)d.w * d.w;
    if (HAS_XT) {
      const float4 t = ld4(x_true, i);
      const double e0 = (double)xn.x - t.x, e1 = (double)xn.y - t.y, e2 = (double)xn.z - t.z, e3 = (double)xn.w - t.w;
      s2 += e0 * e0 + e1 * e1 + e2 * e2 + e3 * e3;
    }
  }
  for (int64_t i = (n4 << 2) + tid; i < n; i += nth) {
    const float d = step * p[i];
    const float xn = x[i] + d;
    x_new[i] = xn;
    s0 += (double)xn * xn;
    s1 += (double)d * d;
    if (HAS_XT) {
      const double e = (double)xn - x_true[i];
      s2 += e * e;
    }
  }
  s0 = block_sum<NT>(s0, lds);
  s1 = block_sum<NT>(s1, lds);
  if (HAS_XT) s2 = block_sum<NT>(s2, lds);
  if (threadIdx.x == 0) {
    partials[blockIdx.x * 3 + 0] = s0;
    partials[blockIdx.x * 3 + 1] = s1;
    partials[blockIdx.x * 3 + 2] = HAS_XT ? s2 : 0.0;
  }
}

template <int C = XS_MAX, class... Args>
void launch_xs(int count, bool has_xt, int grid, hipStream_t s, Args... args) {
  if (count == C) {
    with_bools([&](auto HAS_XT) { hipLaunchKernelGGL((k_cgls_xs_update<HAS_XT, C>), dim3(grid), dim3(NT), 0, s, args...); }, has_xt);
  } else if constexpr (C > 1) {
    launch_xs<C - 1>(count, has_xt, grid, s, args...);
  }
}

}

extern "C" {

int trk_cgls_update_xr(int64_t n, int64_t m, const double* gamma, const double* delta, const float* x, const float* p,
                       float* x_new, float* r, const float* w, const float* x_true, double* sums, trk_stream st) {
  TRK_REQUIRE(gamma && delta && x && p && x_new && r && w && sums, "trk_cgls_update_xr: NULL argument");
  TRK_REQUIRE(n >= 0 && m >= 0, "trk_cgls_update_xr: negative size");
  hipStream_t s = (hipStream_t)st;
  const int grid = stream_grid(n > m ? n : m);
  double* part = nullptr;
  if (int rc = scratch_doubles(s, (size_t)grid * 3, &part)) return rc;
  const bool vec = aligned16(x) && aligned16(p) && aligned16(x_new) && aligned16(r) && aligned16(w) &&
                   (!x_true || aligned16(x_true));
  with_bools([&](auto HAS_XT, auto VEC) {
    hipLaunchKernelGGL((k_cgls_update<HAS_XT, VEC>), dim3(grid), dim3(NT), 0, s, n, m, ScalarSrc{gamma, 1}, ScalarSrc{delta, 1}, x, p, x_new,
                       r, w, x_true, part, (double*)nullptr, stream_nontemporal(n));
  }, x_true != nullptr, vec);
  TRK_LAUNCH_CHECK();
  return finalize_sums(part, grid, 3, 3, sums, s);
}

int trk_cgls_update_xr_deferred(int64_t n, int64_t m, const double* gamma, const double* delta, const float* x,
                                const float* p, float* x_new, float* r, const float* w, const float* x_true,
                                double* norm_partials, int capacity_blocks, int* n_blocks, trk_stream st) {
  return trk_cgls_update_xr_src(n, m, gamma, 1, delta, 1, x, p, x_new, r, w, x_true, nullptr, norm_partials,
                                capacity_blocks, n_blocks, st);
}

int trk_cgls_update_xr_src(int64_t n, int64_t m, const double* gamma, int gamma_n, const double* delta, int delta_n,
                           const float* x, const float* p, float* x_new, float* r, const float* w, const float* x_true,
                           double* publish_delta, double* norm_partials, int capacity_blocks, int* n_blocks,
                           trk_stream st) {
  TRK_REQUIRE(gamma && delta && gamma_n >= 1 && delta_n >= 1 && x && p && x_new && r && w && norm_partials && n_blocks,
              "trk_cgls_update_xr_src: NULL argument");
  TRK_REQUIRE(n >= 0 && m >= 0, "trk_cgls_update_xr_src: negative size");
  hipStream_t s = (hipStream_t)st;
  const int grid = stream_grid(n > m ? n : m);
  TRK_REQUIRE(grid <= capacity_blocks, "trk_cgls_update_xr_src: partial buffer too small (%d blocks needed)", grid);
  *n_blocks = grid;
  const bool vec = aligned16(x) && aligned16(p) && aligned16(x_new) && aligned16(r) && aligned16(w) &&
                   (!x_true || aligned16(x_true));
  const ScalarSrc g{gamma, gamma_n}, d{delta, delta_n};
  with_bools([&](auto HAS_XT, auto VEC) {
    hipLaunchKernelGGL((k_cgls_update<HAS_XT, VEC>), dim3(grid), dim3(NT), 0, s, n, m, g, d, x, p, x_new, r, w, x_true, norm_partials,
                       publish_delta, stream_nontemporal(n));
  }, x_true != nullptr, vec);
  TRK_LAUNCH_CHECK();
  return TRK_OK;
}

int trk_cgls_p_update_to(int64_t n, const float* t, const float* p, float* p_out, const double* gamma_new, int gamma_new_n,
                         const double* gamma_old, double* publish_gamma, trk_stream st) {
  TRK_REQUIRE(t && p && p_out && gamma_new && gamma_new_n >= 1 && gamma_old && n >= 0, "trk_cgls_p_update_to: bad argument");
  const int grid = stream_grid(n);
  const ScalarSrc g{gamma_new, gamma_new_n};
  hipStream_t s = (hipStream_t)st;
  with_bools([&](auto VEC) {
    hipLaunchKernelGGL((k_cgls_p_update<VEC>), dim3(grid), dim3(NT), 0, s, n, t, p, p_out, g, gamma_old, publish_gamma,
                       p == p_out ? 0 : 3);
  }, aligned16(t) && aligned16(p) && aligned16(p_out));
  TRK_LAUNCH_CHECK();
  return TRK_OK;
}

int trk_cgls_p_update(int64_t n, const float* t, float* p, const double* gamma_new, int gamma_new_n,
                      const double* gamma_old, double* publish_gamma, trk_stream st) {
  TRK_REQUIRE(t && p && gamma_new && gamma_new_n >= 1 && gamma_old && n >= 0, "trk_cgls_p_update: bad argument");
  return trk_cgls_p_update_to(n, t, p, p, gamma_new, gamma_new_n, gamma_old, publish_gamma, st);
}

int trk_cgls_r_update(int64_t m, const double* gamma_old, const double* delta, int delta_n, float* r, const float* w,
                      double* publish_delta, trk_stream st) {
  TRK_REQUIRE(gamma_old && delta && delta_n >= 1 && r && w && m >= 0, "trk_cgls_r_update: bad argument");
  const int grid = stream_grid(m);
  const ScalarSrc d{delta, delta_n};
  hipStream_t s = (hipStream_t)st;
  with_bools([&](auto VEC) { hipLaunchKernelGGL((k_cgls_r_update<VEC>), dim3(grid), dim3(NT), 0, s, m, gamma_old, d, r, w, publish_delta); },
             aligned16(r) && aligned16(w));
  TRK_LAUNCH_CHECK();
  return TRK_OK;
}

int trk_cgls_xp_update(int64_t n, const double* gamma_old, const double* delta, const double* gamma_new, int gamma_new_n,
                       const float* x, float* p, const float* t, float* x_new, const float* x_true, double* publish_gamma,
                       double* norm_partials, int capacity_blocks, int* n_blocks, trk_stream st) {
  TRK_REQUIRE(gamma_old && delta && gamma_new && gamma_new_n >= 1 && x && p && t && x_new && norm_partials && n_blocks && n >= 0,
              "trk_cgls_xp_update: bad argument");
  TRK_REQUIRE(aligned16(x) && aligned16(p) && aligned16(t) && aligned16(x_new) && (!x_true || aligned16(x_true)),
              "trk_cgls_xp_update: vectors must be 16-byte aligned");
  const int grid = stream_grid(n);
  TRK_REQUIRE(grid <= capacity_blocks, "trk_cgls_xp_update: partial buffer too small (%d blocks needed)", grid);
  *n_blocks = grid;
  const ScalarSrc g{gamma_new, gamma_new_n};
  hipStream_t s = (hipStream_t)st;
  with_bools([&](auto HAS_XT) {
    hipLaunchKernelGGL((k_cgls_xp_update<HAS_XT>), dim3(grid), dim3(NT), 0, s, n, gamma_old, delta, g, x, p, t, x_new, x_true, publish_gamma,
                       norm_partials, stream_nontemporal(n));
  }, x_true != nullptr);
  TRK_LAUNCH_CHECK();
  return TRK_OK;
}

int trk_cgls_xs_update(int64_t n, int count, int k_last, double* S, const double* gamma_new, int gamma_new_n, const float* x,
                       const float* p, const float* ring, int64_t ring_ld, int s_slots, int first, const float* t, float* x_new,
                       float* p_out, const float* x_true, double* NP, int capacity_blocks, int* n_blocks, trk_stream st) {
  TRK_REQUIRE(S && gamma_new && gamma_new_n >= 1 && x && p && t && x_new && p_out && NP && n_blocks && n >= 0,
              "trk_cgls_xs_update: bad argument");
  TRK_REQUIRE(count >= 1 && count <= XS_MAX && count <= k_last, "trk_cgls_xs_update: need 1 <= count <= %d and count <= k_last", XS_MAX);
  TRK_REQUIRE(s_slots >= count && first >= 0 && first < s_slots && (s_slots == 1 || (ring && ring_ld >= n)),
              "trk_cgls_xs_update: need count <= s_slots, 0 <= first < s_slots and a ring of s_slots - 1 directions");
  XsDirs dirs{};
  for (int c = 0; c < count; ++c) {
    const int slot = (first + c) % s_slots;
    dirs.p[c] = slot == 0 ? p : ring + (int64_t)(slot - 1) * ring_ld;
  }
  bool al = aligned16(x) && aligned16(t) && aligned16(x_new) && aligned16(p_out) && (!x_true || aligned16(x_true));
  for (int c = 0; c < count; ++c) al = al && aligned16(dirs.p[c]);
  TRK_REQUIRE(al, "trk_cgls_xs_update: vectors must be 16-byte aligned");
  const int grid = stream_grid(n);
  TRK_REQUIRE(grid <= capacity_blocks, "trk_cgls_xs_update: partial buffer too small (%d blocks needed)", grid);
  *n_blocks = grid;
  const ScalarSrc g{gamma_new, gamma_new_n};
  hipStream_t s = (hipStream_t)st;
  const int64_t slice = 3 * (int64_t)grid;
  double* part = NP + slice * (k_last - count);
  double* pub = S + 5 * (int64_t)k_last + 1;
  const int nt = stream_nontemporal(n) | (count > 1 ? kXsOldDirs | (p_out == dirs.p[count - 1] ? 0 : kXsLastDirAndOut) : 0);
  launch_xs(count, x_true != nullptr, grid, s, n, (const double*)S, k_last, g, x, dirs, t, x_new, p_out, x_true, pub, part, slice, nt);
  TRK_LAUNCH_CHECK();
  return TRK_OK;
}

int trk_cgls_x_update(int64_t n, const double* gamma, int gamma_n, const double* delta, int delta_n, const float* x,
                      const float* p, float* x_new, const float* x_true, double* publish_delta, double* publish_gamma,
                      double* norm_partials, int capacity_blocks, int* n_blocks, trk_stream st) {
  TRK_REQUIRE(gamma && delta && gamma_n >= 1 && delta_n >= 1 && x && p && x_new && norm_partials && n_blocks,
              "trk_cgls_x_update: NULL argument");
  TRK_REQUIRE(aligned16(x) && aligned16(p) && aligned16(x_new) && (!x_true || aligned16(x_true)),
              "trk_cgls_x_update: vectors must be 16-byte aligned");
  const int grid = stream_grid(n);
  TRK_REQUIRE(grid <= capacity_blocks, "trk_cgls_x_update: partial buffer too small (%d blocks needed)", grid);
  *n_blocks = grid;
  const ScalarSrc g{gamma, gamma_n}, d{delta, delta_n};
  hipStream_t s = (hipStream_t)st;
  with_bools([&](auto HAS_XT) {
    hipLaunchKernelGGL((k_cgls_x_update<HAS_XT>), dim3(grid), dim3(NT), 0, s, n, g, d, x, p, x_new, x_true, publish_delta, publish_gamma,
                       norm_partials);
  }, x_true != nullptr);
  TRK_LAUNCH_CHECK();
  return TRK_OK;
}

}
```

trips_py_amd/csrc/core.hip:

```cpp
#include "trk_internal.h"

#include <algorithm>
#include <cstring>

#include <cstdlib>

#include <cstdarg>
#include <cstdio>
#include <map>
#include <mutex>
#include <vector>

namespace trk {

static thread_local char g_err[512] = "";

void set_error(const char* fmt, ...) {
  va_list ap;
  va_start(ap, fmt);
  vsnprintf(g_err, sizeof g_err, fmt, ap);
  va_end(ap);
}

int fail(int code, const char* fmt, ...) {
// ... 167 lines not shown
  auto* im = new BlockDiagImpl();
  int64_t r = 0, c = 0;
  for (int i = 0; i < count; ++i) {
    if (!ops[i]) {
      delete im;
      return fail(TRK_EINVAL, "trk_blockdiag_create: ops[%d] is NULL", i);
    }
    im->ops.push_back(ops[i]);
    im->roff.push_back(r);
    im->coff.push_back(c);
    r += ops[i]->rows;
    c += ops[i]->cols;
  }
  if (hipMalloc(&im->frame_sums, sizeof(double) * (size_t)count) != hipSuccess) {
    delete im;
    return fail(TRK_ENOMEM, "trk_blockdiag_create: hipMalloc of %d frame sums failed", count);
  }
  auto* op = new trk_op{5, r, c, im, blockdiag_apply, blockdiag_destroy, nullptr, 0};
  *out = op;
  return TRK_OK;
}

int trk_op_shape(const trk_op* op, int64_t* rows, int64_t* cols) {
  TRK_REQUIRE(op, "trk_op_shape: op is NULL");
  if (rows) *rows = op->rows;
  if (cols) *cols = op->cols;
  return TRK_OK;
}

int trk_op_apply(trk_op* op, int transpose, const float* x, int64_t ldx, float* y, int64_t ldy, int batch,
                 double* sumsq_dev, trk_stream stream) {
  TRK_REQUIRE(op && x && y, "trk_op_apply: NULL argument");
  TRK_REQUIRE(batch >= 1, "trk_op_apply: batch must be >= 1 (got %d)", batch);
  const int64_t nin = transpose ? op->rows : op->cols, nout = transpose ? op->cols : op->rows;
  TRK_REQUIRE(batch == 1 || (ldx >= nin && ldy >= nout), "trk_op_apply: ldx/ldy smaller than the vector length");
  TRK_REQUIRE(x != y, "trk_op_apply: in-place apply is not supported");
  return op->apply(op, transpose ? 1 : 0, x, ldx, y, ldy, batch, sumsq_dev, (hipStream_t)stream);
}

int trk_op_axpby_caps(const trk_op* op, int* native) {
  TRK_REQUIRE(op && native, "trk_op_axpby_caps: NULL argument");
  *native = op->apply_axpby ? 1 : 0;
  return TRK_OK;
}

int trk_op_apply_axpby(trk_op* op, int transpose, const float* x, double ca, const double* a_num, const double* a_den,
                       int a_flags, double cb, const double* b_num, const double* b_den, int b_flags, const float* z,
                       float* out, double* sumsq, int hints, trk_stream stream) {
  TRK_REQUIRE(op && x && out, "trk_op_apply_axpby: NULL argument");
  TRK_REQUIRE(out != x && out != z, "trk_op_apply_axpby: out must not alias x or z");
  const int tr = transpose ? 1 : 0;
  if (op->apply_axpby)
    return op->apply_axpby(op, tr, x, Coef{ca, a_num, a_den, a_flags}, Coef{cb, b_num, b_den, b_flags}, z, out, sumsq, hints,
                           (hipStream_t)stream);
  if (op->apply_axpby_plain) {
    const int rc = op->apply_axpby_plain(op, tr, x, Coef{ca, a_num, a_den, a_flags}, Coef{cb, b_num, b_den, b_flags}, z, out, sumsq,
                                         (hipStream_t)stream);
    if (rc != TRK_EUNSUPPORTED) return rc;
  }
  const int64_t nin = tr ? op->rows : op->cols, nout = tr ? op->cols : op->rows;
  if (int rc = op->apply(op, tr, x, nin, out, nout, 1, nullptr, (hipStream_t)stream)) return rc;
  return trk_axpby(nout, ca, a_num, a_den, a_flags, out, cb, b_num, b_den, b_flags, z, out, sumsq, stream);
}

int trk_op_flush(trk_op* op, trk_stream stream) {
  TRK_REQUIRE(op, "trk_op_flush: NULL operator");
  return op->flush ? op->flush(op, (hipStream_t)stream) : TRK_OK;
}

int trk_op_fused_caps(const trk_op* op, int* can_fuse) {
  TRK_REQUIRE(op && can_fuse, "trk_op_fused_caps: NULL argument");
  *can_fuse = op->apply_fused ? op->fused_caps : 0;
  return TRK_OK;
}

int trk_op_apply_fused(trk_op* op, int transpose, const float* x1, const float* x2, double sign, const double* num,
                       int num_n, const double* den, int den_n, float* comb_out, float* y, double* ysq_partials,
                       int capacity, int* n_partials, trk_stream stream) {
  TRK_REQUIRE(op && x1 && y && ysq_partials && n_partials && (!x2 || comb_out), "trk_op_apply_fused: NULL argument");
  TRK_REQUIRE(num_n >= 0 && den_n >= 0 && (num_n == 0 || num) && (den_n == 0 || den), "trk_op_apply_fused: bad scalar source");
  if (!op->apply_fused) return fail(TRK_EUNSUPPORTED, "trk_op_apply_fused: this operator has no fused form");
  return op->apply_fused(op, transpose ? 1 : 0, x1, x2, sign, ScalarSrc{num, num_n}, ScalarSrc{den, den_n}, comb_out, y,
                         ysq_partials, capacity, n_partials, (hipStream_t)stream);
}

int trk_finalize_batched(const double* partials, int nblocks, int nvals, int batches, double* out, int out_stride,
                         trk_stream stream) {
  TRK_REQUIRE(partials && out && nblocks >= 1 && nvals >= 1 && batches >= 0, "trk_finalize_batched: bad argument");
  if (batches == 0) return TRK_OK;
  hipLaunchKernelGGL(k_finalize_batched, dim3(nvals * batches), dim3(256), 0, (hipStream_t)stream, partials, nblocks, nvals,
                     (size_t)nblocks * nvals, nvals, out, out_stride);
  TRK_LAUNCH_CHECK();
  return TRK_OK;
}

int trk_timer_create(int capacity, trk_timer** out) {
  TRK_REQUIRE(out && capacity > 0 && capacity <= (1 << 20), "trk_timer_create: bad capacity");
  auto* t = new trk_timer{new hipEvent_t[2 * (size_t)capacity], capacity, 0};
  for (int i = 0; i < 2 * capacity; ++i) {
    hipError_t e = hipEventCreate(&t->ev[i]);
    if (e != hipSuccess) {
      for (int j = 0; j < i; ++j) (void)hipEventDestroy(t->ev[j]);
      delete[] t->ev;
      delete t;
      return fail(TRK_EHIP, "hipEventCreate: %s", hipGetErrorString(e));
    }
  }
  *out = t;
  return TRK_OK;
}

int trk_timer_reset(trk_timer* t) {
  TRK_REQUIRE(t, "trk_timer_reset: NULL");
  t->used = 0;
  return TRK_OK;
}

int trk_timer_read(trk_timer* t, float* ms_out, int max_out, int* count_out) {
  TRK_REQUIRE(t && ms_out && count_out, "trk_timer_read: NULL argument");
  const int n = t->used < max_out ? t->used : max_out;
  for (int i = 0; i < n; ++i) {
    TRK_HIP(hipEventSynchronize(t->ev[2 * i + 1]));
    TRK_HIP(hipEventElapsedTime(&ms_out[i], t->ev[2 * i], t->ev[2 * i + 1]));
  }
  *count_out = n;
  return TRK_OK;
}

int trk_timer_destroy(trk_timer* t) {
  if (!t) return TRK_OK;
  for (int i = 0; i < 2 * t->cap; ++i) (void)hipEventDestroy(t->ev[i]);
  delete[] t->ev;
  delete t;
  return TRK_OK;
}

int trk_op_set_timer(trk_op* op, trk_timer* t, int which) {
  TRK_REQUIRE(op, "trk_op_set_timer: op is NULL");
  TRK_REQUIRE(which >= 0 && which <= 2, "trk_op_set_timer: which must be 0, 1 or 2");
  op->timer = t;
  op->timer_which = which;
  return TRK_OK;
}

struct trk_mailbox {
  double* host;
  int n;
  unsigned long long* seq;
  unsigned long long* expect;
  hipStream_t* stream;
  unsigned long long counter;
  int slots;
};

namespace {
__global__ void k_mailbox_post(const double* __restrict__ src, double* dst, int count, unsigned long long* seq,
                               unsigned long long value) {
  for (int i = threadIdx.x; i < count; i += blockDim.x) dst[i] = src[i];
  __threadfence_system();
  __syncthreads();
  if (threadIdx.x == 0) {
    __hip_atomic_store(seq, value, __ATOMIC_RELEASE, __HIP_MEMORY_SCOPE_SYSTEM);
  }
}
__global__ void k_mailbox_post_sum(const double* __restrict__ src, double* dst, int count, const double* __restrict__ part, int n,
                                   double* sum_dev, double* sum_host, unsigned long long* seq, unsigned long long value) {
// ... 307 lines not shown
```

trips_py_amd/csrc/trk_internal.h:

```cpp
#pragma once
#include <hip/hip_runtime.h>
#include <stdint.h>
#include <stddef.h>
#include <type_traits>
#include "trk.h"

namespace trk {

void set_error(const char* fmt, ...) __attribute__((format(printf, 1, 2)));
int fail(int code, const char* fmt, ...) __attribute__((format(printf, 2, 3)));

#define TRK_HIP(expr)                                                                         \
  do {                                                                                        \
    hipError_t e_ = (expr);                                                                   \
    if (e_ != hipSuccess) return ::trk::fail(TRK_EHIP, "%s -> %s (%s:%d)", #expr,             \
                                             hipGetErrorString(e_), __FILE__, __LINE__);      \
  } while (0)

#define TRK_REQUIRE(cond, ...)                                  \
  do {                                                          \
    if (!(cond)) return ::trk::fail(TRK_EINVAL, __VA_ARGS__);   \
  } while (0)

#define TRK_LAUNCH_CHECK() TRK_HIP(hipGetLastError())
// ... 145 lines not shown
template <int NV, int N, int OFF>
__device__ __forceinline__ void butterfly_level(double (&v)[NV], int lane) {
  if constexpr (N >= 2) {
#pragma unroll
    for (int i = 0; i < N / 2; ++i) {
      if constexpr (OFF == 32) {
        swap_halves32(v[i], v[i + N / 2]);
        v[i] = v[i] + v[i + N / 2];
      } else if constexpr (OFF == 16) {
        swap_rows16(v[i], v[i + N / 2]);
        v[i] = v[i] + v[i + N / 2];
      } else {
        const bool up = (lane & OFF) != 0;
        const double keep = up ? v[i + N / 2] : v[i], give = up ? v[i] : v[i + N / 2];
        v[i] = keep + lane_xor_f64<OFF>(give);
      }
    }
  } else {
    v[0] = v[0] + lane_xor_f64<OFF>(v[0]);
  }
  if constexpr (OFF > 1) butterfly_level<NV, (N >= 2 ? N / 2 : 1), OFF / 2>(v, lane);
}
template <int NT, int NV>
__device__ __forceinline__ double block_sum_many(const double (&vin)[NV], double* lds) {
  static_assert(NV >= 1 && NV <= 32 && NV <= NT, "at most 32 values, one thread per value");
  constexpr int P = NV <= 8 ? 8 : (NV <= 16 ? 16 : 32);
  constexpr int NW = NT / 64, LPV = 64 / P;
  const int lane = threadIdx.x & 63, wid = threadIdx.x >> 6;
  double v[P];
#pragma unroll
  for (int i = 0; i < P; ++i) v[i] = i < NV ? vin[i < NV ? i : 0] : 0.0;
  butterfly_level<P, P, 32>(v, lane);
  __syncthreads();
  if ((lane & (LPV - 1)) == 0 && lane / LPV < NV) lds[wid * NV + lane / LPV] = v[0];
  __syncthreads();
  double t = 0.0;
  if (threadIdx.x < NV) {
#pragma unroll
    for (int q = 0; q < NW; ++q) t += lds[q * NV + threadIdx.x];
  }
  return t;
}

constexpr int64_t kNontemporalMinFloats = (int64_t)11 << 20;
constexpr int64_t kNontemporalLoadsMinFloats = (int64_t)20 << 20;

struct ScalarSrc {
  const double* p;
  int n;
};

__device__ __forceinline__ double wave_sum_all(double v) {
#pragma unroll
  for (int off = 32; off > 0; off >>= 1) v += __shfl_xor(v, off, 64);
  return v;
}

__device__ __forceinline__ double scalar_from_wave(const ScalarSrc s, int lane) {
  if (s.n == 0) return 1.0;
  if (s.n == 1) return *s.p;
  double a0 = 0.0, a1 = 0.0, a2 = 0.0, a3 = 0.0, a4 = 0.0, a5 = 0.0, a6 = 0.0, a7 = 0.0;
  int i = lane;
  for (; i + 448 < s.n; i += 512) {
    a0 += s.p[i];
    a1 += s.p[i + 64];
    a2 += s.p[i + 128];
    a3 += s.p[i + 192];
    a4 += s.p[i + 256];
    a5 += s.p[i + 320];
    a6 += s.p[i + 384];
    a7 += s.p[i + 448];
  }
  if (i < s.n) a0 += s.p[i];
  if (i + 64 < s.n) a1 += s.p[i + 64];
  if (i + 128 < s.n) a2 += s.p[i + 128];
  if (i + 192 < s.n) a3 += s.p[i + 192];
  if (i + 256 < s.n) a4 += s.p[i + 256];
  if (i + 320 < s.n) a5 += s.p[i + 320];
  if (i + 384 < s.n) a6 += s.p[i + 384];
  double v = ((a0 + a1) + (a2 + a3)) + ((a4 + a5) + (a6 + a7));
  v = wave_sum(v);
  return __hiloint2double(__builtin_amdgcn_readfirstlane(__double2hiint(v)), __builtin_amdgcn_readfirstlane(__double2loint(v)));
}

inline int ceil_div(int64_t a, int64_t b) { return (int)((a + b - 1) / b); }

inline int stream_nontemporal(int64_t n) {
  if (n >= kNontemporalLoadsMinFloats) return 51 | 192;
  return n >= kNontemporalMinFloats ? (3 | 192) : 0;
}

inline bool aligned16(const void* p) { return (reinterpret_cast<uintptr_t>(p) & 15u) == 0; }

template <class F>
inline void with_bools(F&& f) { f(); }
template <class F, class... Rest>
inline void with_bools(F&& f, bool b, Rest... rest) {
  if (b) with_bools([&](auto... c) { f(std::true_type{}, c...); }, rest...);
  else with_bools([&](auto... c) { f(std::false_type{}, c...); }, rest...);
}

}

struct trk_timer {
  hipEvent_t* ev;
  int cap, used;
};

namespace trk {
struct TimerScope {
  trk_timer* t;
  hipStream_t s;
  TimerScope(trk_timer* timer, int which, int transpose, hipStream_t st) : t(nullptr), s(st) {
    if (timer && (which == 2 || which == transpose) && timer->used < timer->cap) {
      t = timer;
      (void)hipEventRecord(t->ev[2 * t->used], s);
    }
  }
  void stop() {
    if (t) {
      (void)hipEventRecord(t->ev[2 * t->used + 1], s);
      ++t->used;
      t = nullptr;
    }
  }
};
}

struct trk_op;
struct PostReq;
namespace trk {
struct RadonRefAngle {
  double inv, dq, k0, w;
  int mode, pad_;
};
struct RadonRefGeom {
  int N, nd, na, nt, npad;
  const RadonRefAngle* ang;
  const unsigned* A32;
  const unsigned* B32;
  int chunk_fwd, chunk_adj;
};
bool radon_ref_geometry(trk_op* op, RadonRefGeom* g);
int radon_ref_apply_f32(const RadonRefGeom& g, int transpose, int weights, const float* x, float* y, hipStream_t s);
int ref_axpby_f32(int64_t n, Coef a, const float* x, Coef b, const float* z, float* out, double* sumsq, hipStream_t s);
int lsqr_damped_update_any(size_t elem_bytes, const void* vk, void* w, const void* x_in, void* x_out, int64_t n, const double* alpha_sq,
                           const double* beta_next_sq, const double* beta0_sq, double damp, const double* state_in, double* state_out,
                           int first, hipStream_t s);
int gemv_t2_partials(const float* V, int64_t ld, int k, int64_t n, const float* r, const float* r2, double** part, int* nblk, hipStream_t s);
int gemv_n_partials(const float* V, int64_t ld, int k, int64_t n, const double* y, double a, const float* base, double sc, float* out,
                    double** part, int* nblk, hipStream_t s);
int scale_by_partials(int64_t n, const double* part, int nblk, const float* x, float* out, double* sum_out, const PostReq& post,
                      hipStream_t s, const float* dotv = nullptr, double* dot_out = nullptr);
int finalize_cgs(const double* part, int nblk, int k, double* W, double* G, int ldg, int passes, double* c, hipStream_t s);
bool blur_separable_params(trk_op* op, int* nx, int* ny, int* kh, int* kw, const float** sep_fwd, const float** sep_adj,
                           int* boundary);
}

struct LsqrReq {
  int on = 0;
  int first = 0;
  float* w = nullptr;
  const float* x_in = nullptr;
  float* x_out = nullptr;
  const float* ref = nullptr;
  double* err_part = nullptr;
  int err_cap = 0;
  const double* a2 = nullptr;
  const double* b2 = nullptr;
  const double* beta0_sq = nullptr;
  double damp = 0.0;
  const double* st_in = nullptr;
  double* st_out = nullptr;
};

struct PostReq {
  int on = 0;
  const double* src = nullptr;
  double* dst = nullptr;
  int count = 0;
  const double* part = nullptr;
  int n_part = 0;
  double* sum_dev = nullptr;
  double* sum_host = nullptr;
  unsigned long long* seq = nullptr;
  unsigned long long value = 0;
};

struct trk_op {
  int kind;
  int64_t rows, cols;
  void* impl;
  int (*apply)(trk_op*, int transpose, const float* x, int64_t ldx, float* y, int64_t ldy, int batch,
               double* sumsq_dev, hipStream_t s);
  void (*destroy)(trk_op*);
  trk_timer* timer = nullptr;
  int timer_which = 0;
  int (*apply_fused)(trk_op*, int transpose, const float* x1, const float* x2, double sign, trk::ScalarSrc num,
                     trk::ScalarSrc den, float* comb, float* y, double* partials, int cap, int* n_partials,
                     hipStream_t s) = nullptr;
  int fused_caps = 1;
  int (*apply_axpby)(trk_op*, int transpose, const float* x, trk::Coef a, trk::Coef b, const float* z, float* out,
                     double* sumsq, int hints, hipStream_t s) = nullptr;
  int (*apply_axpby_plain)(trk_op*, int transpose, const float* x, trk::Coef a, trk::Coef b, const float* z, float* out,
                           double* sumsq, hipStream_t s) = nullptr;
  int (*flush)(trk_op*, hipStream_t s) = nullptr;
  const float* probe_vec = nullptr;
  double* probe_part = nullptr;
  int probe_cap = 0, probe_n = 0;
  LsqrReq lsqr;
  int lsqr_blocks = 0;
  PostReq post;
  int post_taken = 0;
  void* aux = nullptr;
};
```

trips_py_amd/engine.py:

```python
import ctypes

import numpy as np
import torch

from . import _lib

SQRT_NUM = 1
SQRT_DEN = 2


class Coef:

    __slots__ = ("c", "num", "den", "flags", "_keep")

    def __init__(self, c=1.0, num=None, den=None, sqrt_num=False, sqrt_den=False):
        self.c = float(c)
        self.num = _ptr(num)
        self.den = _ptr(den)
        self.flags = (SQRT_NUM if sqrt_num else 0) | (SQRT_DEN if sqrt_den else 0)
        self._keep = (num, den)


_raw_stream = getattr(torch._C, "_cuda_getCurrentRawStream", None)
if _raw_stream is None:
# ... 373 lines not shown
                                                  x_new.data_ptr(), r.data_ptr(), w.data_ptr(),
                                                  None if x_true is None else x_true.data_ptr(), _ptr(partials),
                                                  int(capacity), ctypes.byref(n), self.stream())
        _lib.check(rc, "trk_cgls_update_xr_deferred")
        return n.value

    def op_can_fuse(self, handle):
        can = ctypes.c_int(0)
        _lib.check(self.lib.trk_op_fused_caps(handle, ctypes.byref(can)), "trk_op_fused_caps")
        return can.value

    def op_apply_fused(self, handle, transpose, x1, x2, sign, num, num_n, den, den_n, comb, y, partials, capacity):
        n = ctypes.c_int(0)
        rc = self.lib.trk_op_apply_fused(handle, int(bool(transpose)), x1.data_ptr(), None if x2 is None else x2.data_ptr(),
                                         float(sign), _ptr(num), int(num_n), _ptr(den), int(den_n),
                                         None if comb is None else comb.data_ptr(), y.data_ptr(), _ptr(partials),
                                         int(capacity), ctypes.byref(n), self.stream())
        _lib.check(rc, "trk_op_apply_fused")
        return n.value

    def cgls_update_src(self, gamma, gamma_n, delta, delta_n, x, p, x_new, r, w, x_true, pub_delta, partials, capacity):
        n = ctypes.c_int(0)
        rc = self.lib.trk_cgls_update_xr_src(x.numel(), r.numel(), _ptr(gamma), int(gamma_n), _ptr(delta), int(delta_n),
                                             x.data_ptr(), p.data_ptr(), x_new.data_ptr(), r.data_ptr(), w.data_ptr(),
                                             None if x_true is None else x_true.data_ptr(), _ptr(pub_delta), _ptr(partials),
                                             int(capacity), ctypes.byref(n), self.stream())
        _lib.check(rc, "trk_cgls_update_xr_src")
        return n.value

    def cgls_update_grouping(self, n):
        return int(self.lib.trk_cgls_update_grouping(int(n)))

    def cgls_r_update(self, gamma_old, delta, delta_n, r, w, pub_delta):
        rc = self.lib.trk_cgls_r_update(r.numel(), _ptr(gamma_old), _ptr(delta), int(delta_n), r.data_ptr(), w.data_ptr(),
                                        _ptr(pub_delta), self.stream())
        _lib.check(rc, "trk_cgls_r_update")

    def cgls_xp_update(self, gamma_old, delta, gamma_new, gamma_new_n, x, p, t, x_new, x_true, pub_gamma, partials, capacity):
        n = ctypes.c_int(0)
        rc = self.lib.trk_cgls_xp_update(x.numel(), _ptr(gamma_old), _ptr(delta), _ptr(gamma_new), int(gamma_new_n),
                                         x.data_ptr(), p.data_ptr(), t.data_ptr(), x_new.data_ptr(),
                                         None if x_true is None else x_true.data_ptr(), _ptr(pub_gamma), _ptr(partials),
                                         int(capacity), ctypes.byref(n), self.stream())
        _lib.check(rc, "trk_cgls_xp_update")
        return n.value

    def cgls_p_update(self, t, p, gamma_new, gamma_new_n, gamma_old, pub_gamma):
        rc = self.lib.trk_cgls_p_update(p.numel(), t.data_ptr(), p.data_ptr(), _ptr(gamma_new), int(gamma_new_n),
                                        _ptr(gamma_old), _ptr(pub_gamma), self.stream())
        _lib.check(rc, "trk_cgls_p_update")

    def cgls_x_update(self, gamma, gamma_n, delta, delta_n, x, p, x_new, x_true, pub_delta, pub_gamma, partials, capacity):
        n = ctypes.c_int(0)
        rc = self.lib.trk_cgls_x_update(x.numel(), _ptr(gamma), int(gamma_n), _ptr(delta), int(delta_n), x.data_ptr(),
                                        p.data_ptr(), x_new.data_ptr(), None if x_true is None else x_true.data_ptr(),
                                        _ptr(pub_delta), _ptr(pub_gamma), _ptr(partials), int(capacity), ctypes.byref(n),
                                        self.stream())
        _lib.check(rc, "trk_cgls_x_update")
        return n.value

    def cgls_iterate(self, handle, k_first, n_iters, p, r, t, w, X, keep, x_prev, x_true, S, NP, np_cap, n_np,
                     PG=None, PD=None, pcap=0, grouping=-1):
        c = ctypes.c_int(int(n_np))
        rc = self.lib.trk_cgls_iterate(handle, int(k_first), int(n_iters), p.data_ptr(), r.data_ptr(), t.data_ptr(),
                                       w.data_ptr(), X.data_ptr(), X.stride(0), int(bool(keep)), x_prev.data_ptr(),
                                       None if x_true is None else x_true.data_ptr(), _ptr(S), _ptr(NP), int(np_cap),
                                       ctypes.byref(c), _ptr(PG), _ptr(PD), int(pcap), int(grouping), self.stream())
        _lib.check(rc, "trk_cgls_iterate")
        return c.value

    def cgls_x_batch(self, n):
        return int(self.lib.trk_cgls_x_batch(int(n)))

    def cgls_iterate_xbatch(self, handle, k_first, n_iters, p, ring, s, r, t, w, X, x_prev, x_true, S, NP, np_cap, n_np, PG, PD, pcap):
        c = ctypes.c_int(int(n_np))
        rc = self.lib.trk_cgls_iterate_xbatch(handle, int(k_first), int(n_iters), p.data_ptr(),
                                              None if ring is None else ring.data_ptr(), 0 if ring is None else ring.stride(0),
                                              int(s), r.data_ptr(), t.data_ptr(), w.data_ptr(), X.data_ptr(), X.stride(0),
                                              x_prev.data_ptr(), None if x_true is None else x_true.data_ptr(), _ptr(S), _ptr(NP),
                                              int(np_cap), ctypes.byref(c), _ptr(PG), _ptr(PD), int(pcap), self.stream())
        _lib.check(rc, "trk_cgls_iterate_xbatch")
        return c.value

    def cgls_iterate_fused(self, handle, k_first, n_iters, P, R, t, w, X, keep, x_prev, x_true, S, PG, PD, pcap, NP, np_cap,
                           n_g, n_np):
        cg, cn = ctypes.c_int(int(n_g)), ctypes.c_int(int(n_np))
        rc = self.lib.trk_cgls_iterate_fused(handle, int(k_first), int(n_iters), P.data_ptr(), P.stride(0), R.data_ptr(),
                                             R.stride(0), t.data_ptr(), w.data_ptr(), X.data_ptr(), X.stride(0),
                                             int(bool(keep)), x_prev.data_ptr(), None if x_true is None else x_true.data_ptr(),
                                             _ptr(S), _ptr(PG), _ptr(PD), int(pcap), _ptr(NP), int(np_cap), ctypes.byref(cg),
                                             ctypes.byref(cn), self.stream())
        _lib.check(rc, "trk_cgls_iterate_fused")
        return cg.value, cn.value

    def cgls_tiled_caps(self, handle, np_cap, pcap):
        can = ctypes.c_int(0)
        _lib.check(self.lib.trk_cgls_tiled_caps(handle, int(np_cap), int(pcap), ctypes.byref(can)), "trk_cgls_tiled_caps")
        return bool(can.value)

    def cgls_iterate_tiled(self, handle, k_first, n_iters, P, R, t, X, keep, x_prev, x_true, S, PG, PD, pcap, NP, np_cap,
                           n_g, n_np):
        cg, cn = ctypes.c_int(int(n_g)), ctypes.c_int(int(n_np))
        rc = self.lib.trk_cgls_iterate_tiled(handle, int(k_first), int(n_iters), P.data_ptr(), P.stride(0), R.data_ptr(),
                                             R.stride(0), t.data_ptr(), X.data_ptr(), X.stride(0), int(bool(keep)),
                                             x_prev.data_ptr(), None if x_true is None else x_true.data_ptr(), _ptr(S),
                                             _ptr(PG), _ptr(PD), int(pcap), _ptr(NP), int(np_cap), ctypes.byref(cg),
                                             ctypes.byref(cn), self.stream())
        _lib.check(rc, "trk_cgls_iterate_tiled")
        return cg.value, cn.value

    def cgls_iterate_tiled2(self, handle, k_first, n_iters, p, w, R, t, X, keep, x_prev, x_true, S, PG, PD, pcap, NP, np_cap, n_g, n_np):
        cg, cn = ctypes.c_int(int(n_g)), ctypes.c_int(int(n_np))
        rc = self.lib.trk_cgls_iterate_tiled2(handle, int(k_first), int(n_iters), p.data_ptr(), w.data_ptr(), R.data_ptr(), R.stride(0),
                                              t.data_ptr(), X.data_ptr(), X.stride(0), int(bool(keep)), x_prev.data_ptr(),
                                              None if x_true is None else x_true.data_ptr(), _ptr(S), _ptr(PG), _ptr(PD), int(pcap),
                                              _ptr(NP), int(np_cap), ctypes.byref(cg), ctypes.byref(cn), self.stream())
        _lib.check(rc, "trk_cgls_iterate_tiled2")
        return cg.value, cn.value

    def dot_pair(self, q, w, out3):
        _lib.check(self.lib.trk_dot_pair(q.data_ptr(), None if w is None else w.data_ptr(), q.numel(), _ptr(out3), self.stream()),
                   "trk_dot_pair")

    def cgls_sharded_update(self, G4, gamma_prev, first, x, p, t, x_new, r, q, w, x_true, pub_delta, pub_gamma, partials, capacity):
        n = ctypes.c_int(0)
        rc = self.lib.trk_cgls_sharded_update(x.numel(), r.numel(), _ptr(G4), _ptr(gamma_prev), int(bool(first)),
                                              x.data_ptr(), p.data_ptr(), t.data_ptr(), x_new.data_ptr(), r.data_ptr(), q.data_ptr(),
                                              w.data_ptr(), None if x_true is None else x_true.data_ptr(), _ptr(pub_delta),
                                              _ptr(pub_gamma), _ptr(partials), int(capacity), ctypes.byref(n), self.stream())
        _lib.check(rc, "trk_cgls_sharded_update")
        return n.value

    def cgls_sharded_scalars(self, q, w, gamma_partials, n_gamma, G4):
        rc = self.lib.trk_cgls_sharded_scalars(q.data_ptr(), None if w is None else w.data_ptr(), q.numel(), _ptr(gamma_partials),
                                               int(n_gamma), _ptr(G4), self.stream())
        _lib.check(rc, "trk_cgls_sharded_scalars")

    def cgls_iterate_sharded(self, handle, comm_handle, k_first, n_iters, p, r, t, q, w, X, keep, x_prev, x_true, S, G4, NP, np_cap,
                             n_np, PG=None, pcap=0, n_g=0):
        n = ctypes.c_int(int(n_np))
        ng = ctypes.c_int(int(n_g))
        rc = self.lib.trk_cgls_iterate_sharded(handle, comm_handle, int(k_first), int(n_iters), p.data_ptr(), r.data_ptr(),
                                               t.data_ptr(), q.data_ptr(), w.data_ptr(), X.data_ptr(), X.stride(0), int(keep),
                                               x_prev.data_ptr(), None if x_true is None else x_true.data_ptr(), _ptr(S), _ptr(G4),
                                               _ptr(NP), int(np_cap), ctypes.byref(n), _ptr(PG), int(pcap),
                                               ctypes.byref(ng) if PG is not None else None, self.stream())
        _lib.check(rc, "trk_cgls_iterate_sharded")
        return n.value, ng.value

    def finalize_batched(self, partials, nblocks, nvals, batches, out, out_stride):
        rc = self.lib.trk_finalize_batched(_ptr(partials), int(nblocks), int(nvals), int(batches), _ptr(out), int(out_stride),
                                           self.stream())
        _lib.check(rc, "trk_finalize_batched")

    def gemv_t_x(self, V, k, r, xrow, out_h, out_x):
        rc = self.lib.trk_gemv_t_x(V.data_ptr(), V.stride(0), int(k), r.numel(), r.data_ptr(), xrow.data_ptr(), _ptr(out_h),
                                   _ptr(out_x), self.stream())
        _lib.check(rc, "trk_gemv_t_x")

    def gemv_t(self, V, k, r, out_h, w2=None):
        rc = self.lib.trk_gemv_t(V.data_ptr(), V.stride(0), int(k), r.numel(), r.data_ptr(),
                                 None if w2 is None else w2.data_ptr(), _ptr(out_h), self.stream())
        _lib.check(rc, "trk_gemv_t")

    GEMV_NT_MAX_K = 16

# ... 180 lines not shown
```

trips_py_amd/solvers/CGLS.py:

```python
import numpy as np

from .._io import Formatter, History, as_operator
from ..engine import Coef


class _ShiftedRows:

    def __init__(self, t, shift):
        self.t, self.shift = t, int(shift)

    def data_ptr(self):
        return self.t.data_ptr() + self.shift * self.t.stride(0) * self.t.element_size()

    def stride(self, dim):
        return self.t.stride(dim)

    def row(self, j):
        return self.t[j + self.shift]


def _row_of(X, j, keep):
    if isinstance(X, _ShiftedRows):
        return X.row(j)
    return X[j] if keep else X[j & 1]


class CGLSRun:

    PCAP = 4096
    X_BATCH_MAX = 8

    def __init__(self, A, b, x0, max_iter, x_true=None, history=True, defer_norms=False, grouping=None, x_batch=None):
        self.A = A = as_operator(A)
        self.eng = eng = A.engine
        m, n = A.shape
        self.max_iter = max_iter = int(max_iter)
        self.bv = eng.to_vec(b, m)
        self.xt = None if x_true is None else eng.to_vec(x_true, n)
        x_start = eng.to_vec(x0, n)
        self.hist = History(eng, history, max_iter, n, "CGLS xHistory")
        self.keep = self.hist.keeps_any
        self.X = self.hist.X
        self.defer = bool(defer_norms) and eng.world == 1 and hasattr(eng, "cgls_update_deferred")
        self.NP = eng.scalars(3 * 1024 * max_iter) if self.defer else None
        self.n_np = 0
        self.raw = bool(self.defer and hasattr(eng, "cgls_p_update") and hasattr(A, "_h") and eng.op_can_fuse(A._h))
        self.PG = eng.scalars(self.PCAP) if self.raw else None
        self.PD = eng.scalars(self.PCAP) if self.raw else None
        self.grouping = (int(grouping) if grouping is not None else eng.cgls_update_grouping(n)) if self.raw else 0
        self._final = 0
        self.r, self.t, self.w, self.p = eng.empty(m), eng.empty(n), eng.empty(m), eng.empty(n)
        self.x_batch = 1
        if self.raw and self.grouping == 1 and self.hist.mode == "none" and hasattr(eng, "cgls_iterate_xbatch"):
            self.x_batch = max(1, min(self.X_BATCH_MAX, int(x_batch) if x_batch is not None else eng.cgls_x_batch(n)))
        self.P_ring = eng.empty_basis(self.x_batch - 1, (n + 3) & ~3) if self.x_batch > 1 else None
        self.S = S = eng.scalars(5 * (max_iter + 1))
        self.dist = eng.world > 1
        self.k = 0
        A.apply(x_start, out=self.r)
        eng.axpby(1.0, self.bv, -1.0, self.r, self.r)
        A.apply(self.r, out=self.t, transpose=True, sumsq=S.ref(0))
        eng.allreduce(S, 0, 1)
        self.p.copy_(self.t)
        self.x_cur = x_start

    def slot(self, k):
        return self.X[self.hist.slot(k)]

    def step(self):
        self._step()
        self.hist.pushed(self.k - 1)

    def _run_c_loop(self, n_steps, call):
        h = self.hist
        if h.mode != "stream":
            call(self.k + 1, n_steps, self.X, 1 if h.mode == "device" else 0)
            self.k += n_steps
        else:
            while n_steps > 0:
                k0 = self.k
                c = min(n_steps, h.R // 2, h.R - k0 % h.R)
                for j in range(c):
                    h.row(k0 + j)
                call(k0 + 1, c, _ShiftedRows(self.X, k0 % h.R - k0), 1)
                for j in range(c):
                    h.pushed(k0 + j)
                self.k += c
                n_steps -= c
        self.x_cur = self.slot(self.k - 1)

    def _step(self):
        eng, A, S = self.eng, self.A, self.S
        self.k += 1
        k = self.k
        b = 5 * k
        delta, gamma = S.ref(b), S.ref(b + 1)
        gamma_old = S.ref(0) if k == 1 else S.ref(b - 4)
        x_new = self.hist.row(k - 1)
        if self.raw and self.grouping == 1:
            n_d = eng.op_apply_fused(A._h, False, self.p, None, 0.0, None, 0, None, 0, None, self.w, self.PD.ref(0), self.PCAP)
            eng.cgls_r_update(gamma_old, self.PD.ref(0), n_d, self.r, self.w, delta)
            n_g = eng.op_apply_fused(A._h, True, self.r, None, 0.0, None, 0, None, 0, None, self.t, self.PG.ref(0), self.PCAP)
            self.n_np = eng.cgls_xp_update(gamma_old, delta, self.PG.ref(0), n_g, self.x_cur, self.p, self.t, x_new, self.xt,
                                           gamma, self.NP.ref(3 * self.n_np * (k - 1)), 1024)
            self.x_cur = x_new
            return
        if self.raw:
            n_d = eng.op_apply_fused(A._h, False, self.p, None, 0.0, None, 0, None, 0, None, self.w, self.PD.ref(0), self.PCAP)
            self.n_np = eng.cgls_update_src(gamma_old, 1, self.PD.ref(0), n_d, self.x_cur, self.p, x_new, self.r, self.w,
                                            self.xt, delta, self.NP.ref(3 * self.n_np * (k - 1)), 1024)
            n_g = eng.op_apply_fused(A._h, True, self.r, None, 0.0, None, 0, None, 0, None, self.t, self.PG.ref(0), self.PCAP)
            eng.cgls_p_update(self.t, self.p, self.PG.ref(0), n_g, gamma_old, gamma)
            self.x_cur = x_new
            return
        A.apply(self.p, out=self.w, sumsq=delta)
        if self.dist:
            eng.allreduce(S, b, b + 1)
        if self.defer:
            self.n_np = eng.cgls_update_deferred(gamma_old, delta, self.x_cur, self.p, x_new, self.r, self.w, self.xt,
                                                 self.NP.ref(3 * self.n_np * (k - 1)), 1024)
        else:
            eng.cgls_update(gamma_old, delta, self.x_cur, self.p, x_new, self.r, self.w, self.xt, S.ref(b + 2))
        A.apply(self.r, out=self.t, transpose=True, sumsq=gamma)
        if self.dist:
            eng.allreduce(S, b + 1, b + 5)
        eng.axpby(1.0, self.t, Coef(1.0, num=gamma, den=gamma_old), self.p, self.p)
        self.x_cur = x_new

    def run(self, n_steps):
        n_steps = min(int(n_steps), self.max_iter - self.k)
        if n_steps <= 0:
            return
        eng = self.eng
        if self.defer and not self.dist and hasattr(self.A, "_h") and hasattr(eng, "cgls_iterate"):
            def call(k_first, n, X, keep):
                if self.x_batch > 1:
                    self.n_np = eng.cgls_iterate_xbatch(self.A._h, k_first, n, self.p, self.P_ring, self.x_batch, self.r, self.t,
                                                        self.w, X, self.x_cur, self.xt, self.S.ref(0), self.NP.ref(0), 1024,
                                                        self.n_np, self.PG.ref(0), self.PD.ref(0), self.PCAP)
                    self.x_cur = _row_of(X, k_first + n - 2, keep)
                    return
                self.n_np = eng.cgls_iterate(self.A._h, k_first, n, self.p, self.r, self.t, self.w, X, keep,
                                             self.x_cur, self.xt, self.S.ref(0), self.NP.ref(0), 1024, self.n_np,
                                             None if not self.raw else self.PG.ref(0), None if not self.raw else self.PD.ref(0),
                                             self.PCAP if self.raw else 0, self.grouping)
                self.x_cur = _row_of(X, k_first + n - 2, keep)
            self._run_c_loop(n_steps, call)
        else:
            for _ in range(n_steps):
                self.step()

    def row(self, k):
        return self.S.host(5 * k, 5 * k + 5)

    def rows(self):
        if self.defer and self._final != self.k and self.k > 0:
            self.eng.finalize_batched(self.NP.ref(0), self.n_np, 3, self.k, self.S.ref(7), 5)
            self._final = self.k
        Sh = self.S.host()
        return Sh[0], Sh[5:5 * (self.k + 1)].reshape(self.k, 5)


class CGLSRunSharded(CGLSRun):

    NPC = 1024

    def __init__(self, A, b, x0, max_iter, x_true=None, history=True):
        self.A = A = as_operator(A)
        self.eng = eng = A.engine
        m, n = A.shape
        self.max_iter = max_iter = int(max_iter)
        self.bv = eng.to_vec(b, m)
        self.xt = None if x_true is None else eng.to_vec(x_true, n)
        x_start = eng.to_vec(x0, n)
        self.hist = History(eng, history, max_iter, n, "CGLS xHistory")
        self.keep = self.hist.keeps_any
        self.X = self.hist.X
        self.defer, self.raw, self.grouping, self._final = False, False, 0, 0
        self.NP = eng.scalars(3 * self.NPC * max_iter)
        self.n_np = 0
        self.r, self.t, self.w, self.p, self.q = eng.empty(m), eng.empty(n), eng.zeros(m), eng.zeros(n), eng.empty(m)
        self.S = eng.scalars(5 * (max_iter + 1))
        self.G = eng.scalars(4)
        self.dist = eng.world > 1
        self.k = 0
        self.allreduces = 0
        self._rows = None
        self.rawg = bool(hasattr(eng, "cgls_sharded_scalars") and hasattr(A, "_h") and eng.op_can_fuse(A._h))
        self.PG = eng.scalars(self.PCAP) if self.rawg else None
        self.n_g = 0
        A.apply(x_start, out=self.r)
        eng.axpby(1.0, self.bv, -1.0, self.r, self.r)
        self._adjoint()
        self.x_cur = x_start

    def _adjoint(self):
        if self.rawg:
            self.n_g = self.eng.op_apply_fused(self.A._h, True, self.r, None, 0.0, None, 0, None, 0, None, self.t, self.PG.ref(0),
                                               self.PCAP)
        else:
            self.A.apply(self.r, out=self.t, transpose=True, sumsq=self.G.ref(0))

    def _step(self):
        eng, A, S, G = self.eng, self.A, self.S, self.G
        self.k += 1
        k = self.k
        b = 5 * k
        x_new = self.hist.row(k - 1)
        A.apply(self.t, out=self.q)
        if self.rawg:
            eng.cgls_sharded_scalars(self.q, None if k == 1 else self.w, self.PG.ref(0), self.n_g, G.ref(0))
        else:
            eng.dot_pair(self.q, None if k == 1 else self.w, G.ref(1))
        eng.allreduce(G, 0, 4)
        self.allreduces += self.dist
        self.n_np = eng.cgls_sharded_update(G.ref(0), S.ref(0) if k <= 2 else S.ref(b - 9), k == 1, self.x_cur, self.p,
                                            self.t, x_new, self.r, self.q, self.w, self.xt, S.ref(b),
                                            S.ref(0) if k == 1 else S.ref(b - 4), self.NP.ref(3 * self.n_np * (k - 1)), self.NPC)
# ... 223 lines not shown
```

Measured before the change: 7877 iters/s.

## Add recompute CGLS path that recomputes A*p instead of storing intermediates

Adds a recompute variant of the CGLS iteration for square blur operators of at least 8M elements. A norm-only blur pass computes ||A p||^2 without writing A p. A ratio-epilogue blur pass then recomputes the convolution and fuses the scaled update directly into the output (r or p). This removes the w and t buffer writes and rereads, trading extra stencil arithmetic for less memory traffic on a bandwidth-bound 4096x4096 image.

```diff
diff --git a/include/trk.h b/include/trk.h
--- a/include/trk.h
+++ b/include/trk.h
@@ -169,11 +169,20 @@
 int trk_cgls_xs_update(int64_t n, int count, int k_last, double* S, const double* gamma_new, int gamma_new_n, const float* x,
                        const float* p, const float* ring, int64_t ring_ld, int s_slots, int first, const float* t, float* x_new,
                        float* p_out, const float* x_true, double* NP, int capacity_blocks, int* n_blocks, trk_stream stream);
+int trk_cgls_xs_update_x(int64_t n, int count, int k_last, const double* S, const float* x, const float* p, const float* ring,
+                         int64_t ring_ld, int s_slots, int first, float* x_new, const float* x_true, double* NP,
+                         int capacity_blocks, int* n_blocks, trk_stream stream);
 
 int trk_op_fused_caps(const trk_op* op, int* can_fuse);
 int trk_op_apply_fused(trk_op* op, int transpose, const float* x1, const float* x2, double sign, const double* num,
                        int num_n, const double* den, int den_n, float* comb_out, float* y, double* ysq_partials,
                        int capacity, int* n_partials, trk_stream stream);
+int trk_op_recompute_caps(const trk_op* op, int* can);
+int trk_op_apply_sumsq_raw(trk_op* op, int transpose, const float* x, double* ysq_partials, int capacity, int* n_partials,
+                           trk_stream stream);
+int trk_op_apply_ratio(trk_op* op, int transpose, const float* x, int coef_on_z, double sign, const double* num, int num_n,
+                       const double* den, int den_n, const float* z, float* out, double* publish, int publish_den,
+                       trk_stream stream);
 int trk_cgls_x_update(int64_t n, const double* gamma, int gamma_n, const double* delta, int delta_n, const float* x,
                       const float* p, float* x_new, const float* x_true, double* publish_delta, double* publish_gamma,
                       double* norm_partials, int capacity_blocks, int* n_blocks, trk_stream stream);
@@ -223,6 +232,10 @@
 int trk_cgls_iterate_xbatch(trk_op* A, int k_first, int n_iters, float* p, float* ring, int64_t ring_ld, int s, float* r, float* t,
                             float* w, float* X, int64_t x_ld, const float* x_prev, const float* x_true, double* S, double* NP,
                             int np_capacity_blocks, int* n_np_inout, double* PG, double* PD, int pcap, trk_stream stream);
+int trk_cgls_recompute(int64_t n);
+int trk_cgls_iterate_recompute(trk_op* A, int k_first, int n_iters, float* p, float* ring, int64_t ring_ld, int s, float* r, float* t,
+                               float* w, float* X, int64_t x_ld, const float* x_prev, const float* x_true, double* S, double* NP,
+                               int np_capacity_blocks, int* n_np_inout, double* PG, double* PD, int pcap, trk_stream stream);
 int trk_cgls_iterate_fused(trk_op* A, int k_first, int n_iters, float* P, int64_t p_ld, float* R, int64_t r_ld, float* t,
                            float* w, float* X, int64_t x_ld, int keep_history, const float* x_prev, const float* x_true,
                            double* S, double* PG, double* PD, int pcap, double* NP, int np_capacity_blocks,
diff --git a/trips_py_amd/_lib.py b/trips_py_amd/_lib.py
--- a/trips_py_amd/_lib.py
+++ b/trips_py_amd/_lib.py
@@ -218,6 +218,16 @@
     "trk_cgls_iterate_xbatch": (c_int, [c_op, c_int, c_int, c_f32p, c_f32p, c_i64, c_int, c_f32p, c_f32p, c_f32p, c_f32p, c_i64,
                                         c_f32p, c_f32p, c_f64p, c_f64p, c_int, ctypes.POINTER(c_int), c_f64p, c_f64p, c_int,
                                         c_stream]),
+    "trk_op_recompute_caps": (c_int, [c_op, ctypes.POINTER(c_int)]),
+    "trk_op_apply_sumsq_raw": (c_int, [c_op, c_int, c_f32p, c_f64p, c_int, ctypes.POINTER(c_int), c_stream]),
+    "trk_op_apply_ratio": (c_int, [c_op, c_int, c_f32p, c_int, c_dbl, c_f64p, c_int, c_f64p, c_int, c_f32p, c_f32p, c_f64p, c_int,
+                                   c_stream]),
+    "trk_cgls_xs_update_x": (c_int, [c_i64, c_int, c_int, c_f64p, c_f32p, c_f32p, c_f32p, c_i64, c_int, c_int, c_f32p, c_f32p,
+                                     c_f64p, c_int, ctypes.POINTER(c_int), c_stream]),
+    "trk_cgls_recompute": (c_int, [c_i64]),
+    "trk_cgls_iterate_recompute": (c_int, [c_op, c_int, c_int, c_f32p, c_f32p, c_i64, c_int, c_f32p, c_f32p, c_f32p, c_f32p, c_i64,
+                                           c_f32p, c_f32p, c_f64p, c_f64p, c_int, ctypes.POINTER(c_int), c_f64p, c_f64p, c_int,
+                                           c_stream]),
     "trk_cgls_iterate_fused": (c_int, [c_op, c_int, c_int, c_f32p, c_i64, c_f32p, c_i64, c_f32p, c_f32p, c_f32p, c_i64, c_int,
                                        c_f32p, c_f32p, c_f64p, c_f64p, c_f64p, c_int, c_f64p, c_int, ctypes.POINTER(c_int),
                                        ctypes.POINTER(c_int), c_stream]),
diff --git a/trips_py_amd/csrc/blur2d.hip b/trips_py_amd/csrc/blur2d.hip
--- a/trips_py_amd/csrc/blur2d.hip
+++ b/trips_py_amd/csrc/blur2d.hip
@@ -272,11 +272,25 @@
   Coef a, b;
 };
 
-template <int KH, int KW, int D, bool SUMSQ, bool FUSE, bool EPI = false, int BC = BC_REFLECT>
+enum Rc : int { RC_NONE = 0, RC_NORM = 1, RC_RATIO = 2 };
+struct SlideRatio {
+  const float* z;
+  float* out;
+  ScalarSrc num, den;
+  float sign;
+  int on_z, pub_den;
+  double* pub;
+};
+
+template <int KH, int KW, int D, bool SUMSQ, bool FUSE, bool EPI = false, int BC = BC_REFLECT, int RC = RC_NONE>
 __global__ __launch_bounds__(64) void k_blur_slide(const float* __restrict__ x, int64_t ldx, float* __restrict__ y,
                                                    int64_t ldy, int nx, int ny, const float* __restrict__ wts,
                                                    double* __restrict__ partials, int spans_x, int nbands,
-                                                   int rows_per_band, SlideFuse fz, int nt_store, SlideEpi ep = SlideEpi{}) {
+                                                   int rows_per_band, SlideFuse fz, int nt_store, SlideEpi ep = SlideEpi{},
+                                                   SlideRatio rq = SlideRatio{}) {
+  static_assert(RC == RC_NONE || !FUSE, "the recompute forms take one operand");
+  static_assert(RC != RC_NORM || (SUMSQ && !EPI), "RC_NORM: the sum of squares alone");
+  static_assert(RC != RC_RATIO || (EPI && !SUMSQ), "RC_RATIO: an epilogue form without a sum");
   constexpr int T = KH - 1 - KH / 2;
   constexpr int Lh = KW - 1 - KW / 2;
   constexpr int OFFC = 4 - Lh;
@@ -306,7 +320,7 @@
 
   const unsigned img_bytes = (unsigned)nx * (unsigned)ny * 4u;
   const auto rin = __builtin_amdgcn_make_buffer_rsrc((void*)x, 0, img_bytes, 0x00020000);
-  const auto rout = __builtin_amdgcn_make_buffer_rsrc((void*)y, 0, img_bytes, 0x00020000);
+  const auto rout = __builtin_amdgcn_make_buffer_rsrc((void*)(RC == RC_RATIO ? rq.out : y), 0, img_bytes, 0x00020000);
   const auto rin2 = __builtin_amdgcn_make_buffer_rsrc((void*)(FUSE ? fz.x2 : x), 0, img_bytes, 0x00020000);
   const auto rcomb = __builtin_amdgcn_make_buffer_rsrc((void*)(FUSE ? fz.comb : y), 0, img_bytes, 0x00020000);
   float cb = 0.f;
@@ -358,13 +372,21 @@
   for (int d = 0; d < D; ++d) issue(d, d);
   float ea = 1.f, eb = 0.f;
   f4 zq[EPI ? D : 1];
-  const auto rz = __builtin_amdgcn_make_buffer_rsrc((void*)((EPI && ep.z) ? ep.z : x), 0, img_bytes, 0x00020000);
-  const bool has_z = EPI && ep.z != nullptr;
+  const auto rz = __builtin_amdgcn_make_buffer_rsrc((void*)(RC == RC_RATIO ? rq.z : (EPI && ep.z) ? ep.z : x), 0, img_bytes, 0x00020000);
+  const bool has_z = RC == RC_RATIO || (EPI && ep.z != nullptr);
   auto issue_z = [&](int o, int slot) {
     const int oc = o < band_rows - 1 ? o : band_rows - 1;
     zq[slot] = __builtin_bit_cast(f4, __builtin_amdgcn_raw_buffer_load_b128(rz, vc, (ofirst + dir * oc) * rowbytes, 0));
   };
-  if (EPI) {
+  if constexpr (RC == RC_RATIO) {
+#pragma unroll
+    for (int d = 0; d < D; ++d) issue_z(d, d);
+    const double qn = scalar_from_wave(rq.num, lane), qd = scalar_from_wave(rq.den, lane);
+    const float c = rq.sign * (float)(qn / qd);
+    ea = rq.on_z ? 1.f : c;
+    eb = rq.on_z ? c : 1.f;
+    if (blockIdx.x == 0 && blockIdx.y == 0 && lane == 0 && rq.pub) *rq.pub = rq.pub_den ? qd : qn;
+  } else if (EPI) {
     ea = (float)coef_eval(ep.a);
     eb = has_z ? (float)coef_eval(ep.b) : 0.f;
     if (has_z) {
@@ -442,7 +464,17 @@
         f4 out = (f4){acc[kd][0][0], acc[kd][0][1], acc[kd][1][0], acc[kd][1][1]};
         if (EPI) {
           const int zs = pmod(u - (KH - 1), D);
-          if (has_z) {
+          if constexpr (RC == RC_RATIO) {
+            const f4 zv = zq[zs];
+            if (rq.on_z) {
+#pragma unroll
+              for (int e = 0; e < 4; ++e) out[e] = fmaf(eb, zv[e], out[e]);
+            } else {
+#pragma unroll
+              for (int e = 0; e < 4; ++e) out[e] = fmaf(ea, out[e], zv[e]);
+            }
+            issue_z(o + D, zs);
+          } else if (has_z) {
             const f4 zv = zq[zs];
 #pragma unroll
             for (int e = 0; e < 4; ++e) out[e] = fmaf(ea, out[e], eb * zv[e]);
@@ -453,10 +485,12 @@
           }
         }
         if (active) {
-          if (nt_store & 1)
-            __builtin_amdgcn_raw_buffer_store_b128(__builtin_bit_cast(u4, out), rout, vst + (ofirst + dir * o) * rowbytes, 0, 2);
-          else
-            __builtin_amdgcn_raw_buffer_store_b128(__builtin_bit_cast(u4, out), rout, vst + (ofirst + dir * o) * rowbytes, 0, 0);
+          if constexpr (RC != RC_NORM) {
+            if (nt_store & 1)
+              __builtin_amdgcn_raw_buffer_store_b128(__builtin_bit_cast(u4, out), rout, vst + (ofirst + dir * o) * rowbytes, 0, 2);
+            else
+              __builtin_amdgcn_raw_buffer_store_b128(__builtin_bit_cast(u4, out), rout, vst + (ofirst + dir * o) * rowbytes, 0, 0);
+          }
           if (SUMSQ) qacc = fmaf(out[0], out[0], fmaf(out[1], out[1], fmaf(out[2], out[2], fmaf(out[3], out[3], qacc))));
         }
       }
@@ -539,23 +573,23 @@
   const float* w = im->sep_dev[tr];
   const int nts = stream_nontemporal((int64_t)im->nx * im->ny);
   if (fuse) {
-    hipExtLaunchKernelGGL((k_blur_slide<K, K, D, true, true, false, BC>), grid, block, 0, s, ev0, ev1, 0, x, ldx, y, ldy, im->nx, im->ny, w, part, spans_x, nbands, rows_per_band, *fuse, nts, SlideEpi{});
+    hipExtLaunchKernelGGL((k_blur_slide<K, K, D, true, true, false, BC>), grid, block, 0, s, ev0, ev1, 0, x, ldx, y, ldy, im->nx, im->ny, w, part, spans_x, nbands, rows_per_band, *fuse, nts, SlideEpi{}, SlideRatio{});
     TRK_LAUNCH_CHECK();
     return TRK_OK;
   }
   const SlideFuse nofuse{nullptr, nullptr, 0.0, {nullptr, 0}, {nullptr, 0}};
   if (epi) {
     if (part)
-      hipExtLaunchKernelGGL((k_blur_slide<K, K, D, true, false, true, BC>), grid, block, 0, s, ev0, ev1, 0, x, ldx, y, ldy, im->nx, im->ny, w, part, spans_x, nbands, rows_per_band, nofuse, nts, *epi);
+      hipExtLaunchKernelGGL((k_blur_slide<K, K, D, true, false, true, BC>), grid, block, 0, s, ev0, ev1, 0, x, ldx, y, ldy, im->nx, im->ny, w, part, spans_x, nbands, rows_per_band, nofuse, nts, *epi, SlideRatio{});
     else
-      hipExtLaunchKernelGGL((k_blur_slide<K, K, D, false, false, true, BC>), grid, block, 0, s, ev0, ev1, 0, x, ldx, y, ldy, im->nx, im->ny, w, part, spans_x, nbands, rows_per_band, nofuse, nts, *epi);
+      hipExtLaunchKernelGGL((k_blur_slide<K, K, D, false, false, true, BC>), grid, block, 0, s, ev0, ev1, 0, x, ldx, y, ldy, im->nx, im->ny, w, part, spans_x, nbands, rows_per_band, nofuse, nts, *epi, SlideRatio{});
     TRK_LAUNCH_CHECK();
     return TRK_OK;
   }
   if (part)
-    hipExtLaunchKernelGGL((k_blur_slide<K, K, D, true, false, false, BC>), grid, block, 0, s, ev0, ev1, 0, x, ldx, y, ldy, im->nx, im->ny, w, part, spans_x, nbands, rows_per_band, nofuse, nts, SlideEpi{});
+    hipExtLaunchKernelGGL((k_blur_slide<K, K, D, true, false, false, BC>), grid, block, 0, s, ev0, ev1, 0, x, ldx, y, ldy, im->nx, im->ny, w, part, spans_x, nbands, rows_per_band, nofuse, nts, SlideEpi{}, SlideRatio{});
   else
-    hipExtLaunchKernelGGL((k_blur_slide<K, K, D, false, false, false, BC>), grid, block, 0, s, ev0, ev1, 0, x, ldx, y, ldy, im->nx, im->ny, w, part, spans_x, nbands, rows_per_band, nofuse, nts, SlideEpi{});
+    hipExtLaunchKernelGGL((k_blur_slide<K, K, D, false, false, false, BC>), grid, block, 0, s, ev0, ev1, 0, x, ldx, y, ldy, im->nx, im->ny, w, part, spans_x, nbands, rows_per_band, nofuse, nts, SlideEpi{}, SlideRatio{});
   TRK_LAUNCH_CHECK();
   return TRK_OK;
 }
@@ -736,6 +770,61 @@
   return TRK_OK;
 }
 
+template <int K, int D, int BC>
+int launch_slide_rc(const BlurImpl* im, int tr, const float* x, double* part, const SlideRatio* rq, int spans_x, int nbands,
+                    int rows_per_band, hipStream_t s, hipEvent_t ev0, hipEvent_t ev1) {
+  dim3 grid(spans_x * nbands, 1), block(64);
+  const float* w = im->sep_dev[tr];
+  const SlideFuse nofuse{nullptr, nullptr, 0.0, {nullptr, 0}, {nullptr, 0}};
+  if (rq)
+    hipExtLaunchKernelGGL((k_blur_slide<K, K, D, false, false, true, BC, RC_RATIO>), grid, block, 0, s, ev0, ev1, 0, x, 0, rq->out, 0, im->nx, im->ny, w, part, spans_x, nbands, rows_per_band, nofuse, 0, SlideEpi{}, *rq);
+  else
+    hipExtLaunchKernelGGL((k_blur_slide<K, K, D, true, false, false, BC, RC_NORM>), grid, block, 0, s, ev0, ev1, 0, x, 0, (float*)nullptr, 0, im->nx, im->ny, w, part, spans_x, nbands, rows_per_band, nofuse, 0, SlideEpi{}, SlideRatio{});
+  TRK_LAUNCH_CHECK();
+  return TRK_OK;
+}
+
+int blur_apply_rc(trk_op* op, int tr, const float* x, double* partials, int cap, int* n_partials, const SlideRatio* rq, hipStream_t s) {
+  auto* im = static_cast<BlurImpl*>(op->impl);
+  if (!slide_shape_ok(im) || !aligned16(x) || (rq && (!aligned16(rq->z) || !aligned16(rq->out))))
+    return fail(TRK_EUNSUPPORTED, "blur2d recompute forms: need a separable odd PSF <= 9x9, ny %% 4 == 0, 16-byte aligned buffers");
+  if (rq && (rq->out == x || rq->z == x))
+    return fail(TRK_EINVAL, "blur2d ratio apply: out / z must not alias x (halo rows are shared)");
+  int spans_x, nbands, rpb;
+  const int Usel = (im->kh == 9) ? 9 : (im->kh == 7) ? 7 : (im->kh == 5) ? 5 : 6;
+  slide_grid(im->nx, im->ny, 1, im->kh, Usel, &spans_x, &nbands, &rpb);
+  if (!rq) {
+    const int nblk = spans_x * nbands;
+    if (nblk > cap) return fail(TRK_EINVAL, "blur2d norm-only apply: partial buffer holds %d doubles, %d needed", cap, nblk);
+    *n_partials = nblk;
+  }
+  hipEvent_t ev0 = nullptr, ev1 = nullptr;
+  if (trk_timer* t = op->timer)
+    if (rq && (op->timer_which == 2 || op->timer_which == tr) && t->used < t->cap) {
+      ev0 = t->ev[2 * t->used];
+      ev1 = t->ev[2 * t->used + 1];
+      ++t->used;
+    }
+  return bc_dispatch(im->bc, [&](auto bc) {
+    constexpr int BC = decltype(bc)::value;
+    switch (im->kh) {
+      case 3: return launch_slide_rc<3, 6, BC>(im, tr, x, partials, rq, spans_x, nbands, rpb, s, ev0, ev1);
+      case 5: return launch_slide_rc<5, 5, BC>(im, tr, x, partials, rq, spans_x, nbands, rpb, s, ev0, ev1);
+      case 7: return launch_slide_rc<7, 7, BC>(im, tr, x, partials, rq, spans_x, nbands, rpb, s, ev0, ev1);
+      default: return launch_slide_rc<9, 9, BC>(im, tr, x, partials, rq, spans_x, nbands, rpb, s, ev0, ev1);
+    }
+  });
+}
+
+int blur_apply_norm(trk_op* op, int tr, const float* x, double* partials, int cap, int* n_partials, hipStream_t s) {
+  return blur_apply_rc(op, tr, x, partials, cap, n_partials, nullptr, s);
+}
+
+int blur_apply_ratio(trk_op* op, int tr, const float* x, const RatioCoef& c, const float* z, float* out, hipStream_t s) {
+  const SlideRatio rq{z, out, c.num, c.den, (float)c.sign, c.on_z, c.pub_den, c.pub};
+  return blur_apply_rc(op, tr, x, nullptr, 0, nullptr, &rq, s);
+}
+
 void blur_destroy(trk_op* op) {
   auto* im = static_cast<BlurImpl*>(op->impl);
   for (int t = 0; t < 2; ++t) {
@@ -839,6 +928,10 @@
   auto* op = new trk_op{1, n, n, im, blur_apply, blur_destroy, nullptr, 0};
   if (slide_shape_ok(im)) op->apply_fused = blur_apply_fused;
   if (slide_shape_ok(im)) op->apply_axpby_plain = blur_apply_axpby_plain;
+  if (slide_shape_ok(im)) {
+    op->apply_norm = blur_apply_norm;
+    op->apply_ratio = blur_apply_ratio;
+  }
   *out = op;
   return TRK_OK;
 }
diff --git a/trips_py_amd/csrc/cgls_loop.hip b/trips_py_amd/csrc/cgls_loop.hip
--- a/trips_py_amd/csrc/cgls_loop.hip
+++ b/trips_py_amd/csrc/cgls_loop.hip
@@ -114,6 +114,56 @@
   return TRK_OK;
 }
 
+int trk_cgls_recompute(int64_t n) {
+  return n >= ((int64_t)8 << 20) ? 1 : 0;
+}
+
+int trk_cgls_iterate_recompute(trk_op* A, int k_first, int n_iters, float* p, float* ring, int64_t ring_ld, int s, float* r, float* t,
+                               float* w, float* X, int64_t x_ld, const float* x_prev, const float* x_true, double* S, double* NP,
+                               int np_capacity_blocks, int* n_np_inout, double* PG, double* PD, int pcap, trk_stream stream) {
+  (void)t;
+  (void)w;
+  TRK_REQUIRE(A && p && r && X && x_prev && S && NP && n_np_inout && PG && PD && pcap > 0, "trk_cgls_iterate_recompute: NULL argument");
+  TRK_REQUIRE(A->apply_norm && A->apply_ratio, "trk_cgls_iterate_recompute: the operator has no recompute forms (trk_op_recompute_caps)");
+  TRK_REQUIRE(A->rows == A->cols, "trk_cgls_iterate_recompute: square operators only");
+  TRK_REQUIRE(k_first >= 1 && n_iters >= 0, "trk_cgls_iterate_recompute: need k_first >= 1, n_iters >= 0");
+  TRK_REQUIRE(s >= 1 && (s == 1 || (ring && ring_ld >= A->cols)), "trk_cgls_iterate_recompute: s > 1 needs a ring of s - 1 directions");
+  const int64_t n = A->cols;
+  int n_np = *n_np_inout;
+  auto slot = [&](int j) { return j == 0 ? p : ring + (int64_t)(j - 1) * ring_ld; };
+  int cur = 0, pending = 0;
+  const int k_end = k_first + n_iters;
+  for (int k = k_first; k < k_end; ++k) {
+    double* row = S + 5 * (int64_t)k;
+    const double* gamma_old = (k == 1) ? S : row - 4;
+    float* p_k = slot(cur);
+    int n_d = 0, n_g = 0;
+    int rc = trk_op_apply_sumsq_raw(A, 0, p_k, PD, pcap, &n_d, stream);
+    if (rc) return rc;
+    rc = trk_op_apply_ratio(A, 0, p_k, 0, -1.0, gamma_old, 1, PD, n_d, r, r, row, 1, stream);
+    if (rc) return rc;
+    const bool last = k + 1 == k_end;
+    const bool batch = ++pending >= s || last;
+    if (batch) {
+      float* x_new = X + (int64_t)((k - 1) & 1) * x_ld;
+      rc = trk_cgls_xs_update_x(n, pending, k, S, x_prev, p, ring, ring_ld, s, (cur - pending + 1 + s) % s, x_new, x_true, NP,
+                                np_capacity_blocks, &n_np, stream);
+      if (rc) return rc;
+      x_prev = x_new;
+      pending = 0;
+    }
+    rc = trk_op_apply_sumsq_raw(A, 1, r, PG, pcap, &n_g, stream);
+    if (rc) return rc;
+    float* p_next = batch ? (last ? p : p_k) : slot((cur + 1) % s);
+    rc = trk_op_apply_ratio(A, 1, r, 1, 1.0, PG, n_g, gamma_old, 1, p_k, p_next, row + 1, 0, stream);
+    if (rc) return rc;
+    if (!batch) cur = (cur + 1) % s;
+    if (last) cur = 0;
+  }
+  *n_np_inout = n_np;
+  return TRK_OK;
+}
+
 int trk_cgls_iterate_fused(trk_op* A, int k_first, int n_iters, float* P, int64_t p_ld, float* R, int64_t r_ld, float* t,
                            float* w, float* X, int64_t x_ld, int keep_history, const float* x_prev, const float* x_true,
                            double* S, double* PG, double* PD, int pcap, double* NP, int np_capacity_blocks,
diff --git a/trips_py_amd/csrc/cgls_update.hip b/trips_py_amd/csrc/cgls_update.hip
--- a/trips_py_amd/csrc/cgls_update.hip
+++ b/trips_py_amd/csrc/cgls_update.hip
@@ -217,7 +217,7 @@
   const float* p[XS_MAX];
 };
 
-template <bool HAS_XT, int C>
+template <bool HAS_XT, int C, bool XONLY = false>
 __global__ __launch_bounds__(NT) void k_cgls_xs_update(int64_t n, const double* S, int k, ScalarSrc gnew, const float* x, XsDirs dirs,
                                                        const float* __restrict__ t, float* x_new, float* p_out,
                                                        const float* __restrict__ x_true, double* pub_gamma,
@@ -225,7 +225,7 @@
   __shared__ double lds[NT / 64];
   __shared__ double bc[C + 1];
   if (threadIdx.x < 64) {
-    const double g = scalar_from_wave(gnew, threadIdx.x);
+    const double g = XONLY ? 0.0 : scalar_from_wave(gnew, threadIdx.x);
     if (threadIdx.x == 0) {
 #pragma unroll
       for (int c = 0; c < C; ++c) {
@@ -233,15 +233,17 @@
         const double* gold = (j == 1) ? S : S + 5 * (int64_t)(j - 1) + 1;
         bc[c] = *gold / S[5 * (int64_t)j];
       }
-      bc[C] = g / *((k == 1) ? S : S + 5 * (int64_t)(k - 1) + 1);
-      if (blockIdx.x == 0 && pub_gamma) *pub_gamma = g;
+      if (!XONLY) {
+        bc[C] = g / *((k == 1) ? S : S + 5 * (int64_t)(k - 1) + 1);
+        if (blockIdx.x == 0 && pub_gamma) *pub_gamma = g;
+      }
     }
   }
   __syncthreads();
   float step[C];
 #pragma unroll
   for (int c = 0; c < C; ++c) step[c] = (float)bc[c];
-  const float b = (float)bc[C];
+  const float b = XONLY ? 0.f : (float)bc[C];
   double s0[C], s1[C], s2[C];
 #pragma unroll
   for (int c = 0; c < C; ++c) s0[c] = s1[c] = s2[c] = 0.0;
@@ -252,7 +254,8 @@
     float4 pv[C];
 #pragma unroll
     for (int c = 0; c < C; ++c) pv[c] = (nt & (c < C - 1 ? 256 : 512)) ? ld4_nt(dirs.p[c], i) : ld4(dirs.p[c], i);
-    const float4 tv = (nt & 32) ? ld4_nt(t, i) : ld4(t, i);
+    float4 tv = make_float4(0.f, 0.f, 0.f, 0.f);
+    if (!XONLY) tv = (nt & 32) ? ld4_nt(t, i) : ld4(t, i);
     const float4 tt = HAS_XT ? ld4(x_true, i) : make_float4(0.f, 0.f, 0.f, 0.f);
 #pragma unroll
     for (int c = 0; c < C; ++c) {
@@ -261,14 +264,16 @@
       x_norms4<HAS_XT>(xv, d, tt, s0[c], s1[c], s2[c]);
     }
     if (nt & 2) st4_nt(x_new, i, xv); else st4(x_new, i, xv);
-    if (nt & 1024) st4_nt(p_out, i, p_step4(tv, pv[C - 1], b)); else st4(p_out, i, p_step4(tv, pv[C - 1], b));
+    if (!XONLY) {
+      if (nt & 1024) st4_nt(p_out, i, p_step4(tv, pv[C - 1], b)); else st4(p_out, i, p_step4(tv, pv[C - 1], b));
+    }
   }
   for (int64_t i = (n4 << 2) + tid; i < n; i += nth) {
     float xv = x[i];
     float pv[C];
 #pragma unroll
     for (int c = 0; c < C; ++c) pv[c] = dirs.p[c][i];
-    const float tv = t[i], tt = HAS_XT ? x_true[i] : 0.f;
+    const float tv = XONLY ? 0.f : t[i], tt = HAS_XT ? x_true[i] : 0.f;
 #pragma unroll
     for (int c = 0; c < C; ++c) {
       float d;
@@ -276,7 +281,7 @@
       x_norms<HAS_XT>(xv, d, tt, s0[c], s1[c], s2[c]);
     }
     x_new[i] = xv;
-    p_out[i] = fmaf(1.f, tv, b * pv[C - 1]);
+    if (!XONLY) p_out[i] = fmaf(1.f, tv, b * pv[C - 1]);
   }
 #pragma unroll
   for (int c = 0; c < C; ++c) {
@@ -356,6 +361,14 @@
     launch_xs<C - 1>(count, has_xt, grid, s, args...);
   }
 }
+template <int C = XS_MAX, class... Args>
+void launch_xs_x(int count, bool has_xt, int grid, hipStream_t s, Args... args) {
+  if (count == C) {
+    with_bools([&](auto HAS_XT) { hipLaunchKernelGGL((k_cgls_xs_update<HAS_XT, C, true>), dim3(grid), dim3(NT), 0, s, args...); }, has_xt);
+  } else if constexpr (C > 1) {
+    launch_xs_x<C - 1>(count, has_xt, grid, s, args...);
+  }
+}
 
 }
 
@@ -490,6 +503,34 @@
   return TRK_OK;
 }
 
+int trk_cgls_xs_update_x(int64_t n, int count, int k_last, const double* S, const float* x, const float* p, const float* ring,
+                         int64_t ring_ld, int s_slots, int first, float* x_new, const float* x_true, double* NP,
+                         int capacity_blocks, int* n_blocks, trk_stream st) {
+  TRK_REQUIRE(S && x && p && x_new && NP && n_blocks && n >= 0, "trk_cgls_xs_update_x: bad argument");
+  TRK_REQUIRE(count >= 1 && count <= XS_MAX && count <= k_last, "trk_cgls_xs_update_x: need 1 <= count <= %d and count <= k_last", XS_MAX);
+  TRK_REQUIRE(s_slots >= count && first >= 0 && first < s_slots && (s_slots == 1 || (ring && ring_ld >= n)),
+              "trk_cgls_xs_update_x: need count <= s_slots, 0 <= first < s_slots and a ring of s_slots - 1 directions");
+  XsDirs dirs{};
+  for (int c = 0; c < count; ++c) {
+    const int slot = (first + c) % s_slots;
+    dirs.p[c] = slot == 0 ? p : ring + (int64_t)(slot - 1) * ring_ld;
+  }
+  bool al = aligned16(x) && aligned16(x_new) && (!x_true || aligned16(x_true));
+  for (int c = 0; c < count; ++c) al = al && aligned16(dirs.p[c]);
+  TRK_REQUIRE(al, "trk_cgls_xs_update_x: vectors must be 16-byte aligned");
+  const int grid = stream_grid(n);
+  TRK_REQUIRE(grid <= capacity_blocks, "trk_cgls_xs_update_x: partial buffer too small (%d blocks needed)", grid);
+  *n_blocks = grid;
+  hipStream_t s = (hipStream_t)st;
+  const int64_t slice = 3 * (int64_t)grid;
+  double* part = NP + slice * (k_last - count);
+  const int nt = (stream_nontemporal(n) & ~32) | (count > 1 ? 256 : 0);
+  launch_xs_x(count, x_true != nullptr, grid, s, n, S, k_last, ScalarSrc{nullptr, 0}, x, dirs, (const float*)nullptr, x_new,
+              (float*)nullptr, x_true, (double*)nullptr, part, slice, nt);
+  TRK_LAUNCH_CHECK();
+  return TRK_OK;
+}
+
 int trk_cgls_x_update(int64_t n, const double* gamma, int gamma_n, const double* delta, int delta_n, const float* x,
                       const float* p, float* x_new, const float* x_true, double* publish_delta, double* publish_gamma,
                       double* norm_partials, int capacity_blocks, int* n_blocks, trk_stream st) {
diff --git a/trips_py_amd/csrc/core.hip b/trips_py_amd/csrc/core.hip
--- a/trips_py_amd/csrc/core.hip
+++ b/trips_py_amd/csrc/core.hip
@@ -273,6 +273,30 @@
   if (!op->apply_fused) return fail(TRK_EUNSUPPORTED, "trk_op_apply_fused: this operator has no fused form");
   return op->apply_fused(op, transpose ? 1 : 0, x1, x2, sign, ScalarSrc{num, num_n}, ScalarSrc{den, den_n}, comb_out, y,
                          ysq_partials, capacity, n_partials, (hipStream_t)stream);
+}
+
+int trk_op_recompute_caps(const trk_op* op, int* can) {
+  TRK_REQUIRE(op && can, "trk_op_recompute_caps: NULL argument");
+  *can = (op->apply_norm && op->apply_ratio) ? 1 : 0;
+  return TRK_OK;
+}
+
+int trk_op_apply_sumsq_raw(trk_op* op, int transpose, const float* x, double* ysq_partials, int capacity, int* n_partials,
+                           trk_stream stream) {
+  TRK_REQUIRE(op && x && ysq_partials && n_partials && capacity > 0, "trk_op_apply_sumsq_raw: bad argument");
+  if (!op->apply_norm) return fail(TRK_EUNSUPPORTED, "trk_op_apply_sumsq_raw: this operator has no norm-only form (trk_op_recompute_caps)");
+  return op->apply_norm(op, transpose ? 1 : 0, x, ysq_partials, capacity, n_partials, (hipStream_t)stream);
+}
+
+int trk_op_apply_ratio(trk_op* op, int transpose, const float* x, int coef_on_z, double sign, const double* num, int num_n,
+                       const double* den, int den_n, const float* z, float* out, double* publish, int publish_den,
+                       trk_stream stream) {
+  TRK_REQUIRE(op && x && z && out && num && den && num_n >= 1 && den_n >= 1, "trk_op_apply_ratio: bad argument");
+  TRK_REQUIRE(sign == 1.0 || sign == -1.0, "trk_op_apply_ratio: sign must be +1 or -1");
+  TRK_REQUIRE(out != x && z != x, "trk_op_apply_ratio: out / z must not alias x");
+  if (!op->apply_ratio) return fail(TRK_EUNSUPPORTED, "trk_op_apply_ratio: this operator has no ratio form (trk_op_recompute_caps)");
+  const RatioCoef c{ScalarSrc{num, num_n}, ScalarSrc{den, den_n}, sign, coef_on_z ? 1 : 0, publish_den ? 1 : 0, publish};
+  return op->apply_ratio(op, transpose ? 1 : 0, x, c, z, out, (hipStream_t)stream);
 }
 
 int trk_finalize_batched(const double* partials, int nblocks, int nvals, int batches, double* out, int out_stride,
diff --git a/trips_py_amd/csrc/trk_internal.h b/trips_py_amd/csrc/trk_internal.h
--- a/trips_py_amd/csrc/trk_internal.h
+++ b/trips_py_amd/csrc/trk_internal.h
@@ -251,6 +251,13 @@
   v = wave_sum(v);
   return __hiloint2double(__builtin_amdgcn_readfirstlane(__double2hiint(v)), __builtin_amdgcn_readfirstlane(__double2loint(v)));
 }
+
+struct RatioCoef {
+  ScalarSrc num, den;
+  double sign;
+  int on_z, pub_den;
+  double* pub;
+};
 
 inline int ceil_div(int64_t a, int64_t b) { return (int)((a + b - 1) / b); }
 
@@ -373,6 +380,9 @@
                      double* sumsq, int hints, hipStream_t s) = nullptr;
   int (*apply_axpby_plain)(trk_op*, int transpose, const float* x, trk::Coef a, trk::Coef b, const float* z, float* out,
                            double* sumsq, hipStream_t s) = nullptr;
+  int (*apply_norm)(trk_op*, int transpose, const float* x, double* partials, int cap, int* n_partials, hipStream_t s) = nullptr;
+  int (*apply_ratio)(trk_op*, int transpose, const float* x, const trk::RatioCoef& c, const float* z, float* out,
+                     hipStream_t s) = nullptr;
   int (*flush)(trk_op*, hipStream_t s) = nullptr;
   const float* probe_vec = nullptr;
   double* probe_part = nullptr;
diff --git a/trips_py_amd/engine.py b/trips_py_amd/engine.py
--- a/trips_py_amd/engine.py
+++ b/trips_py_amd/engine.py
@@ -479,6 +479,37 @@
         _lib.check(rc, "trk_cgls_iterate_xbatch")
         return c.value
 
+    def op_can_recompute(self, handle):
+        can = ctypes.c_int(0)
+        _lib.check(self.lib.trk_op_recompute_caps(handle, ctypes.byref(can)), "trk_op_recompute_caps")
+        return can.value
+
+    def op_apply_sumsq_raw(self, handle, transpose, x, partials, capacity):
+        n = ctypes.c_int(0)
+        rc = self.lib.trk_op_apply_sumsq_raw(handle, int(bool(transpose)), x.data_ptr(), _ptr(partials), int(capacity),
+                                             ctypes.byref(n), self.stream())
+        _lib.check(rc, "trk_op_apply_sumsq_raw")
+        return n.value
+
+    def op_apply_ratio(self, handle, transpose, x, coef_on_z, sign, num, num_n, den, den_n, z, out, publish=None, publish_den=False):
+        rc = self.lib.trk_op_apply_ratio(handle, int(bool(transpose)), x.data_ptr(), int(bool(coef_on_z)), float(sign), _ptr(num),
+                                         int(num_n), _ptr(den), int(den_n), z.data_ptr(), out.data_ptr(), _ptr(publish),
+                                         int(bool(publish_den)), self.stream())
+        _lib.check(rc, "trk_op_apply_ratio")
+
+    def cgls_recompute(self, n):
+        return int(self.lib.trk_cgls_recompute(int(n)))
+
+    def cgls_iterate_recompute(self, handle, k_first, n_iters, p, ring, s, r, X, x_prev, x_true, S, NP, np_cap, n_np, PG, PD, pcap):
+        c = ctypes.c_int(int(n_np))
+        rc = self.lib.trk_cgls_iterate_recompute(handle, int(k_first), int(n_iters), p.data_ptr(),
+                                                 None if ring is None else ring.data_ptr(), 0 if ring is None else ring.stride(0),
+                                                 int(s), r.data_ptr(), None, None, X.data_ptr(), X.stride(0),
+                                                 x_prev.data_ptr(), None if x_true is None else x_true.data_ptr(), _ptr(S), _ptr(NP),
+                                                 int(np_cap), ctypes.byref(c), _ptr(PG), _ptr(PD), int(pcap), self.stream())
+        _lib.check(rc, "trk_cgls_iterate_recompute")
+        return c.value
+
     def cgls_iterate_fused(self, handle, k_first, n_iters, P, R, t, w, X, keep, x_prev, x_true, S, PG, PD, pcap, NP, np_cap,
                            n_g, n_np):
         cg, cn = ctypes.c_int(int(n_g)), ctypes.c_int(int(n_np))
diff --git a/trips_py_amd/solvers/CGLS.py b/trips_py_amd/solvers/CGLS.py
--- a/trips_py_amd/solvers/CGLS.py
+++ b/trips_py_amd/solvers/CGLS.py
@@ -30,7 +30,8 @@
     PCAP = 4096
     X_BATCH_MAX = 8
 
-    def __init__(self, A, b, x0, max_iter, x_true=None, history=True, defer_norms=False, grouping=None, x_batch=None):
+    def __init__(self, A, b, x0, max_iter, x_true=None, history=True, defer_norms=False, grouping=None, x_batch=None,
+                 recompute=None):
         self.A = A = as_operator(A)
         self.eng = eng = A.engine
         m, n = A.shape
@@ -51,8 +52,11 @@
         self._final = 0
         self.r, self.t, self.w, self.p = eng.empty(m), eng.empty(n), eng.empty(m), eng.empty(n)
         self.x_batch = 1
+        self.recompute = False
         if self.raw and self.grouping == 1 and self.hist.mode == "none" and hasattr(eng, "cgls_iterate_xbatch"):
             self.x_batch = max(1, min(self.X_BATCH_MAX, int(x_batch) if x_batch is not None else eng.cgls_x_batch(n)))
+            if m == n and hasattr(eng, "cgls_iterate_recompute") and eng.op_can_recompute(A._h):
+                self.recompute = bool(eng.cgls_recompute(n)) if recompute is None else bool(recompute)
         self.P_ring = eng.empty_basis(self.x_batch - 1, (n + 3) & ~3) if self.x_batch > 1 else None
         self.S = S = eng.scalars(5 * (max_iter + 1))
         self.dist = eng.world > 1
@@ -134,6 +138,12 @@
         eng = self.eng
         if self.defer and not self.dist and hasattr(self.A, "_h") and hasattr(eng, "cgls_iterate"):
             def call(k_first, n, X, keep):
+                if self.recompute:
+                    self.n_np = eng.cgls_iterate_recompute(self.A._h, k_first, n, self.p, self.P_ring, self.x_batch, self.r, X,
+                                                           self.x_cur, self.xt, self.S.ref(0), self.NP.ref(0), 1024, self.n_np,
+                                                           self.PG.ref(0), self.PD.ref(0), self.PCAP)
+                    self.x_cur = _row_of(X, k_first + n - 2, keep)
+                    return
                 if self.x_batch > 1:
                     self.n_np = eng.cgls_iterate_xbatch(self.A._h, k_first, n, self.p, self.P_ring, self.x_batch, self.r, self.t,
                                                         self.w, X, self.x_cur, self.xt, self.S.ref(0), self.NP.ref(0), 1024,
```

New measurement: 8529 iters/s (median of 6 runs). 8.3% higher.
